# j-min/HiREST

Hardware: AMD Instinct MI355X
Metric: encoded frames/sec (EVA-CLIP-g/14 224^2) (higher is better)
Workload: dtype bf16

## Files before the change

### hirest_amd/_lib.py

```python
from __future__ import annotations

import ctypes as C
import os

HERE = os.path.dirname(os.path.abspath(__file__))
LIB_PATH = os.path.join(HERE, "lib", "libhirest_hip.so")
if os.environ.get("HIREST_LIB_VARIANT"):
    LIB_PATH = os.path.join(HERE, "lib", f"libhirest_hip.{os.environ['HIREST_LIB_VARIANT']}.so")

(EPI_BIAS_BF16, EPI_BIAS_GELU_BF16, EPI_BIAS_QGELU_BF16, EPI_BIAS_RESID_F32, EPI_BIAS_F32, EPI_PATCH_POS_F32,
 EPI_BIAS_RESID_LNSTATS_F32, EPI_LNFOLD_BF16, EPI_LNFOLD_GELU_BF16, EPI_BIAS_GELU_SPLIT2, EPI_BIAS_RESID2_LNSTATS) = range(11)

TOWER_NO_LNFOLD = 1
TOWER_NO_PRUNE = 2
TOWER_F32_RESIDUAL = 4
GEMM_REVERSE = 1
GEMM_X3 = 2
GEMM_X3_T128 = 4
ABI_VERSION = 4

ERRORS = {-1: "HIREST_E_BADARG", -2: "HIREST_E_SHAPE (unsupported shape)", -3: "HIREST_E_WORKSPACE (workspace too small)"}


class GemmArgs(C.Structure):
    _fields_ = [("struct_size", C.c_uint64),
                ("A", C.c_void_p), ("lda", C.c_int64), ("W", C.c_void_p), ("ldw", C.c_int64),
                ("bias", C.c_void_p), ("out", C.c_void_p), ("ldo", C.c_int64),
                ("M", C.c_int32), ("N", C.c_int32), ("K", C.c_int32), ("epilogue", C.c_int32),
                ("pos", C.c_void_p), ("patches_per_frame", C.c_int32), ("aux0", C.c_void_p), ("aux1", C.c_void_p), ("flags", C.c_int32)]

    @classmethod
    def make(cls, *fields):
        return cls(C.sizeof(cls), *fields)



class BlockWeights(C.Structure):
    _fields_ = [(n, C.c_void_p) for n in ("ln1_g", "ln1_b", "qkv_w", "qkv_b", "proj_w", "proj_b",
                                          "ln2_g", "ln2_b", "fc1_w", "fc1_b", "fc2_w", "fc2_b",
                                          "qkv_wf", "qkv_bf", "qkv_s", "fc1_wf", "fc1_bf", "fc1_s")]


class VisionTower(C.Structure):
    _fields_ = [(n, C.c_int32) for n in ("image_size", "patch", "width", "heads", "head_dim", "mlp_dim",
                                         "layers", "embed_dim", "kpad", "act")] + \
               [("ln_eps", C.c_float)] + \
               [("patch_w", C.c_void_p), ("patch_b", C.c_void_p), ("cls", C.c_void_p), ("pos", C.c_void_p),
                ("blocks", C.POINTER(BlockWeights)),
                ("norm_g", C.c_void_p), ("norm_b", C.c_void_p), ("head_w", C.c_void_p), ("head_b", C.c_void_p),
                ("image_mean", C.c_void_p), ("image_std", C.c_void_p),
                ("ln_pre_g", C.c_void_p), ("ln_pre_b", C.c_void_p), ("out_all_tokens", C.c_int32)]


class TextTower(C.Structure):
    _fields_ = [(n, C.c_int32) for n in ("context", "vocab", "width", "heads", "layers", "embed_dim", "act")] + \
               [("ln_eps", C.c_float)] + \
               [("tok_emb", C.c_void_p), ("pos", C.c_void_p), ("blocks", C.POINTER(BlockWeights)),
                ("lnf_g", C.c_void_p), ("lnf_b", C.c_void_p), ("proj_w", C.c_void_p)]


class BlockWeightsF32(C.Structure):
    _fields_ = [(n, C.c_void_p) for n in ("ln1_g", "ln1_b", "qkv_w", "qkv_b", "proj_w", "proj_b",
                                          "ln2_g", "ln2_b", "fc1_w", "fc1_b", "fc2_w", "fc2_b")]


class VisionTowerF32(C.Structure):
    _fields_ = [(n, t) if n != "blocks" else (n, C.POINTER(BlockWeightsF32)) for n, t in VisionTower._fields_]


class TextTowerF32(C.Structure):
    _fields_ = [(n, t) if n != "blocks" else (n, C.POINTER(BlockWeightsF32)) for n, t in TextTower._fields_]


class BlockWeightsX3(C.Structure):
    _fields_ = [(n, C.c_void_p) for n in ("qkv_w2", "proj_w2", "fc1_w2", "fc2_w2")]


class VisionTowerX3(C.Structure):
    _fields_ = [("base", C.POINTER(VisionTowerF32)), ("blocks", C.POINTER(BlockWeightsX3))]


class CaptionLayer(C.Structure):
    _fields_ = [(n, C.c_void_p) for n in ("qkv_w", "qkv_b", "so_w", "so_b", "so_ln_g", "so_ln_b", "cq_w", "cq_b",
                                          "co_w", "co_b", "co_ln_g", "co_ln_b", "ff1_w", "ff1_b", "ff2_w", "ff2_b", "ff_ln_g", "ff_ln_b")]


class CaptionDecoder(C.Structure):
    _fields_ = [(n, C.c_int32) for n in ("layers", "heads", "hidden", "inter", "vocab_padded", "max_pos")] + \
               [(n, C.c_void_p) for n in ("word_emb", "pos_emb", "emb_ln_g", "emb_ln_b")] + \
               [("layer", C.POINTER(CaptionLayer))] + \
               [(n, C.c_void_p) for n in ("tr_w", "tr_b", "tr_ln_g", "tr_ln_b", "lm_w", "lm_b", "lm_w2")]


class JointLayerX3(C.Structure):
    _fields_ = [(n, C.c_void_p) for n in ("qkv_w2", "qkv_b", "ao_w2", "ao_b", "ln1_g", "ln1_b", "fc1_w2", "fc1_b", "fc2_w2", "fc2_b", "ln2_g", "ln2_b")]


class JointEncoderX3(C.Structure):
    _fields_ = [("struct_size", C.c_uint64)] + [(n, C.c_int32) for n in ("layers", "heads", "width", "mlp_dim", "in_dim", "max_pos")] + \
               [("ln_eps", C.c_float), ("attn_shift", C.c_float)] + \
               [(n, C.c_void_p) for n in ("emb_w2", "emb_b", "pos", "emb_ln_g", "emb_ln_b")] + [("layer", C.POINTER(JointLayerX3))]


class ColsumItem(C.Structure):
    _fields_ = [("x", C.c_void_p), ("row_weight", C.c_void_p), ("row_select", C.c_void_p), ("out", C.c_void_p), ("ldx", C.c_int64),
                ("R", C.c_int32), ("C", C.c_int32), ("select_value", C.c_int32), ("reserved", C.c_int32)]


COLSUM_GROUP_MAX = 40


class SplitItem(C.Structure):
    _fields_ = [("x", C.c_void_p), ("out", C.c_void_p), ("ldx", C.c_int64), ("ldo", C.c_int64), ("rows", C.c_int32), ("cols", C.c_int32),
                ("transposed", C.c_int32), ("reserved", C.c_int32)]


class OptimItem(C.Structure):
    _fields_ = [("p", C.c_void_p), ("g", C.c_void_p), ("m", C.c_void_p), ("v", C.c_void_p), ("n", C.c_int64)]


OPTIM_GROUP_MAX = 64
OPTIM_CHUNK = 8192


class TrainBlock(C.Structure):
    _fields_ = [("struct_size", C.c_uint64)] + [(n, C.c_int32) for n in ("B", "T", "heads", "width", "mlp", "precision")] + \
               [("ln_eps", C.c_float), ("drop", C.c_float)] + [(n, C.c_uint32) for n in ("seed_attn", "seed_ao", "seed_out", "reserved")] + \
               [(n, C.c_void_p) for n in ("wqkv", "bqkv", "wo", "bo", "ln1_g", "ln1_b", "w1", "b1", "w2", "b2", "ln2_g", "ln2_b", "x",
                                          "qkv", "P", "cx", "a_pre", "aa", "hpre", "hh", "x_pre", "out", "x2", "out2",
                                          "wqkv2", "wo2", "w12", "w22", "wqkvT2", "woT2", "w1T2", "w2T2", "ws")] + [("ws_bytes", C.c_size_t)]


class TrainFusionBwd(C.Structure):
    _fields_ = [("struct_size", C.c_uint64)] + \
               [(n, C.c_int32) for n in ("B", "T", "E", "W", "vis_dim", "text_dim", "asr_dim", "boundary", "max_pos", "reserved")] + \
               [("drop", C.c_float), ("seed_emb", C.c_uint32)] + \
               [(n, C.c_void_p) for n in ("w_emb", "emb_ln_g", "t2_w", "asr1_w", "asr0_g", "norm_g",
                                          "x0", "f", "v", "tn", "tin", "a0", "asr2", "v0", "vis2", "t", "text", "mm32", "bm32", "n_valid", "dx",
                                          "g_emb_ln_g", "g_emb_ln_b", "g_pos", "g_w_emb", "g_b_emb", "g_mask", "g_bound", "g_t2_w", "g_t2_b", "g_t0_w", "g_t0_b",
                                          "g_asr1_w", "g_asr1_b", "g_asr0_g", "g_asr0_b", "g_norm_g", "g_norm_b", "g_vis_w", "g_vis_b", "g_text_w", "g_text_b")] + \
               [("items", C.POINTER(ColsumItem)), ("n_items", C.POINTER(C.c_int32)), ("max_items", C.c_int32), ("reserved2", C.c_int32),
                ("ws", C.c_void_p), ("ws_bytes", C.c_size_t), ("side_stream", C.c_void_p), ("side_ws", C.c_void_p), ("side_ws_bytes", C.c_size_t),
                ("scratch", C.c_void_p), ("scratch_bytes", C.c_size_t)]


class TrainBlockGrads(C.Structure):
    _fields_ = [("struct_size", C.c_uint64)] + \
               [(n, C.c_void_p) for n in ("dout", "dx", "g_wqkv", "g_wo", "g_w1", "g_w2", "g_bqkv", "g_bo", "g_b1", "g_b2", "g_ln1_g", "g_ln1_b",
                                          "g_ln2_g", "g_ln2_b")] + \
               [("items", C.POINTER(ColsumItem)), ("n_items", C.POINTER(C.c_int32)), ("max_items", C.c_int32), ("reserved", C.c_int32),
                ("side_stream", C.c_void_p), ("side_ws", C.c_void_p), ("side_ws_bytes", C.c_size_t), ("scratch", C.c_void_p),
                ("scratch_bytes", C.c_size_t)]


class JpegImage(C.Structure):
    _fields_ = [(n, C.c_int32) for n in ("width", "height", "ncomp", "hs", "vs", "restart_interval", "mcux", "mcuy", "supported",
                                         "reason")] + \
               [("scan_begin", C.c_int64), ("scan_end", C.c_int64), ("table_set", C.c_int32), ("reserved", C.c_int32),
                ("data_offset", C.c_int64), ("out_offset", C.c_int64), ("ws_offset", C.c_int64),
                ("plane_offset", C.c_int64)]


class JpegTables(C.Structure):
    _fields_ = [("qt", (C.c_uint16 * 64) * 3), ("huff_bits", (C.c_uint8 * 16) * 6), ("huff_vals", (C.c_uint8 * 256) * 6)]


JPEG_REASONS = {0: "ok", 1: "not a JPEG / malformed markers", 2: "progressive", 3: "arithmetic coding", 4: "lossless / hierarchical",
                5: "not 8-bit", 6: "colour space (CMYK / YCCK / RGB / component count)", 7: "sampling factors", 8: "multi-scan",
                9: "truncated (no EOI after the scan)", 10: "bad or missing tables", 11: "image size"}
JPEG_STATUS = {1: "bad Huffman code", 2: "more than 64 coefficients in a block", 4: "out of data", 8: "RSTn out of sequence",
               16: "unsupported"}


BATCH_GATHER_MAX = 8


class BatchGather(C.Structure):
    _fields_ = [("src", C.c_void_p), ("dst", C.c_void_p), ("row_of_example", C.c_void_p), ("words", C.c_int32), ("reserved", C.c_int32)]


class BatchArgs(C.Structure):
    _fields_ = [("struct_size", C.c_uint64), ("index", C.c_void_p)] + \
               [(n, C.c_int32) for n in ("B", "T", "D", "Da", "n_examples", "n_model_frames", "n_gather", "reserved")] + \
               [(n, C.c_void_p) for n in ("frames", "frame_off", "asr_rows", "sub_off", "sub_span", "ex_video", "ex_len", "ex_range",
                                          "bound_off", "bound_val", "vis", "asr", "vis_mask", "moment_mask", "prev_boundary_mask")] + \
               [("gather", BatchGather * BATCH_GATHER_MAX)]


class ProfRecord(C.Structure):
    _fields_ = [("kind", C.c_int32), ("tag", C.c_int32), ("d0", C.c_int64), ("d1", C.c_int64), ("d2", C.c_int64),
                ("ms", C.c_float)]


_SIGNATURES = {
    "hirest_profile_enable": (C.c_int, [C.c_int32]),
    "hirest_attention_debug_mode": (C.c_int, [C.c_int32]),
    "hirest_profile_collect": (C.c_int, [C.POINTER(ProfRecord), C.c_int32]),
    "hirest_abi_version": (C.c_int, []),
    "hirest_build_info": (C.c_char_p, []),
    "hirest_gemm_bf16": (C.c_int, [C.POINTER(GemmArgs), C.c_void_p]),
    "hirest_gemm_select_kernel": (C.c_int, [C.c_int32]),
    "hirest_gemm_debug_mode": (C.c_int, [C.c_int32]),
    "hirest_gemm_dispatch_name": (C.c_int, [C.POINTER(GemmArgs), C.c_char_p, C.c_int32]),
    "hirest_attention_select_kernel": (C.c_int, [C.c_int32]),
    "hirest_attention_set_skew": (C.c_int, [C.c_int32]),
    "hirest_attention_set_mapping": (C.c_int, [C.c_int32]),
    "hirest_attention_set_pace": (C.c_int, [C.c_int32]),
    "hirest_attention_x3_select_waves": (C.c_int, [C.c_int32]),
    "hirest_attention_x3_debug_trace": (C.c_int, [C.c_void_p]),
    "hirest_attention_set_stagger": (C.c_int, [C.c_int32]),
    "hirest_attention_debug_trace_read": (C.c_int, [C.c_void_p, C.c_int32]),
    "hirest_layernorm": (C.c_int, [C.c_void_p, C.c_int64, C.c_void_p, C.c_void_p, C.c_void_p, C.c_float,
                                   C.c_void_p, C.c_int64, C.c_int32, C.c_int32, C.c_int32, C.c_void_p]),
    "hirest_attention_bf16": (C.c_int, [C.c_void_p, C.c_void_p, C.c_int32, C.c_int32, C.c_int32, C.c_int32,
                                        C.c_float, C.c_int32, C.c_void_p]),
    "hirest_attention_bf16_rows": (C.c_int, [C.c_void_p, C.c_void_p, C.c_int32, C.c_int32, C.c_int32, C.c_int32,
                                             C.c_float, C.c_int32, C.c_int32, C.c_void_p]),
    "hirest_fold_layernorm": (C.c_int, [C.c_void_p, C.c_void_p, C.c_void_p, C.c_void_p, C.c_void_p, C.c_void_p, C.c_void_p, C.c_int32,
                                        C.c_int32, C.c_void_p]),
    "hirest_patchify": (C.c_int, [C.c_void_p, C.c_int32, C.c_int32, C.c_int32, C.c_int32, C.c_void_p, C.c_void_p,
                                  C.c_void_p, C.c_int32, C.c_void_p]),
    "hirest_rowstats_bf16": (C.c_int, [C.c_void_p, C.c_int64, C.c_void_p, C.c_void_p, C.c_float, C.c_int32, C.c_int32, C.c_void_p, C.c_void_p]),
    "hirest_rowstats_split_bf16": (C.c_int, [C.c_void_p, C.c_int64, C.c_void_p, C.c_void_p, C.c_void_p, C.c_float, C.c_int32, C.c_int32, C.c_void_p,
                                             C.c_void_p]),
    "hirest_combine_hi_lo_f32": (C.c_int, [C.c_void_p, C.c_void_p, C.c_int64, C.c_void_p, C.c_int64, C.c_int32, C.c_int32, C.c_void_p]),
    "hirest_ln_stats_finalize": (C.c_int, [C.c_void_p, C.c_int32, C.c_void_p, C.c_float, C.c_int32, C.c_int32, C.c_void_p, C.c_void_p]),
    "hirest_write_cls_rows": (C.c_int, [C.c_void_p, C.c_int64, C.c_void_p, C.c_void_p, C.c_int32, C.c_int32,
                                        C.c_int32, C.c_void_p]),
    "hirest_embed_tokens": (C.c_int, [C.c_void_p, C.c_void_p, C.c_void_p, C.c_void_p, C.c_void_p, C.c_int32,
                                      C.c_int32, C.c_int32, C.c_int32, C.c_void_p]),
    "hirest_f32_to_bf16": (C.c_int, [C.c_void_p, C.c_void_p, C.c_int64, C.c_void_p]),
    "hirest_pool_l2norm": (C.c_int, [C.c_void_p, C.c_void_p, C.c_int32, C.c_int32, C.c_int32, C.c_int32, C.c_void_p]),
    "hirest_pool_l2norm_varlen": (C.c_int, [C.c_void_p, C.c_void_p, C.c_void_p, C.c_int32, C.c_int32, C.c_void_p]),
    "hirest_similarity_f32": (C.c_int, [C.c_void_p, C.c_void_p, C.c_void_p, C.c_int32, C.c_int32, C.c_int32, C.c_void_p]),
    "hirest_topk_workspace_bytes": (C.c_int64, [C.c_int32, C.c_int32, C.c_int32]),
    "hirest_topk_f32_ws": (C.c_int, [C.c_void_p, C.c_void_p, C.c_int32, C.c_int32, C.c_int32, C.c_void_p, C.c_void_p, C.c_void_p,
                                     C.c_int64, C.c_void_p]),
    "hirest_topk_f32": (C.c_int, [C.c_void_p, C.c_void_p, C.c_int32, C.c_int32, C.c_int32, C.c_void_p, C.c_void_p,
                                  C.c_void_p]),
    "hirest_clip_score": (C.c_int, [C.c_void_p, C.c_int32, C.c_int32, C.c_void_p, C.c_int32, C.c_void_p, C.c_int32, C.c_int32,
                                    C.c_int32, C.c_void_p, C.c_void_p]),
    "hirest_bertscore_greedy": (C.c_int, [C.c_void_p, C.c_int64, C.c_int32, C.c_void_p, C.c_int32, C.c_void_p, C.c_void_p, C.c_void_p,
                                          C.c_int32, C.c_void_p, C.c_void_p]),
    "hirest_gemm_f32": (C.c_int, [C.c_void_p, C.c_int64, C.c_void_p, C.c_int64, C.c_void_p, C.c_void_p, C.c_int64, C.c_void_p,
                                  C.c_int32, C.c_void_p, C.c_int64, C.c_int32, C.c_int32, C.c_int32, C.c_int32, C.c_void_p]),
    "hirest_attention_f32": (C.c_int, [C.c_void_p, C.c_void_p, C.c_int32, C.c_int32, C.c_int32, C.c_int32, C.c_float,
                                       C.c_float, C.c_void_p]),
    "hirest_attention_f32_qkv": (C.c_int, [C.c_void_p, C.c_int64, C.c_void_p, C.c_void_p, C.c_int64, C.c_void_p, C.c_int32, C.c_int32,
                                           C.c_int32, C.c_int32, C.c_int32, C.c_float, C.c_float, C.c_float, C.c_void_p]),
    "hirest_gemm_f32_select_kernel": (C.c_int, [C.c_int32]),
    "hirest_gemm_f32_workspace_bytes": (C.c_size_t, [C.c_int32, C.c_int32, C.c_int32]),
    "hirest_gemm_f32_layouts_workspace_bytes": (C.c_size_t, [C.c_int32, C.c_int32, C.c_int32]),
    "hirest_gemm_f32_layouts": (C.c_int, [C.c_void_p, C.c_int64, C.c_int32, C.c_void_p, C.c_int64, C.c_int32, C.c_void_p, C.c_void_p, C.c_int64,
                                          C.c_void_p, C.c_int64, C.c_int32, C.c_int32, C.c_int32, C.c_int32, C.c_void_p, C.c_size_t, C.c_void_p]),
    "hirest_gemm_f32_ws": (C.c_int, [C.c_void_p, C.c_int64, C.c_void_p, C.c_int64, C.c_void_p, C.c_void_p, C.c_int64, C.c_void_p,
                                     C.c_int32, C.c_void_p, C.c_int64, C.c_int32, C.c_int32, C.c_int32, C.c_int32, C.c_void_p, C.c_size_t,
                                     C.c_void_p]),
    "hirest_attention_f32_decode": (C.c_int, [C.c_void_p, C.c_int64, C.c_void_p, C.c_void_p, C.c_int64, C.c_void_p, C.c_int32, C.c_void_p,
                                              C.c_void_p, C.c_int64, C.c_void_p, C.c_void_p, C.c_void_p, C.c_int32, C.c_int32, C.c_float,
                                              C.c_float, C.c_float, C.c_void_p]),
    "hirest_gemm_f32_ln": (C.c_int, [C.c_void_p, C.c_int64, C.c_void_p, C.c_void_p, C.c_void_p, C.c_void_p, C.c_void_p, C.c_float,
                                     C.c_void_p, C.c_int64, C.c_void_p, C.c_int64, C.c_void_p, C.c_void_p, C.c_int64, C.c_void_p,
                                     C.c_int64, C.c_int32, C.c_int32, C.c_int32, C.c_int32, C.c_void_p]),
    "hirest_caption_step_workspace_bytes": (C.c_size_t, [C.POINTER(CaptionDecoder), C.c_int32]),
    "hirest_beam_backtrack": (C.c_int, [C.c_void_p, C.c_void_p, C.c_void_p, C.c_void_p, C.c_int32, C.c_int32, C.c_int32, C.c_void_p, C.c_void_p]),
    "hirest_beam_advance": (C.c_int, [C.c_void_p, C.c_void_p, C.c_int32, C.c_int32, C.c_int32, C.c_int32, C.c_int32, C.c_int32,
                                      C.c_void_p, C.c_void_p, C.c_void_p, C.c_void_p, C.c_void_p, C.c_void_p, C.c_void_p, C.c_void_p,
                                      C.c_void_p]),
    "hirest_caption_decode_step": (C.c_int, [C.POINTER(CaptionDecoder), C.c_int32, C.c_int32, C.c_void_p, C.c_void_p,
                                             C.POINTER(C.c_void_p), C.POINTER(C.c_void_p), C.POINTER(C.c_void_p), C.c_int32,
                                             C.c_void_p, C.c_void_p, C.c_void_p, C.c_size_t, C.c_void_p]),
    "hirest_caption_decode_logits": (C.c_int, [C.POINTER(CaptionDecoder), C.c_int32, C.c_int32, C.c_void_p, C.c_void_p,
                                               C.POINTER(C.c_void_p), C.POINTER(C.c_void_p), C.POINTER(C.c_void_p), C.c_int32,
                                               C.c_void_p, C.c_void_p, C.c_size_t, C.c_void_p]),
    "hirest_caption_select": (C.c_int, [C.c_int32]),
    "hirest_gemm_f32_ln_colmax": (C.c_int, [C.c_void_p, C.c_int64, C.c_void_p, C.c_void_p, C.c_float, C.c_void_p, C.c_int64, C.c_void_p,
                                            C.c_void_p, C.c_int64, C.c_void_p, C.c_int32, C.c_int32, C.c_int32, C.c_void_p]),
    "hirest_gemm_f32_rows_ln_mode": (C.c_int, [C.c_int32]),
    "hirest_gemm_f32_ring_mode": (C.c_int, [C.c_int32]),
    "hirest_gemm_f32_rows_preferred": (C.c_int, [C.c_int32]),
    "hirest_gemm_f32_rows_colmax": (C.c_int, [C.c_void_p, C.c_int64, C.c_void_p, C.c_int64, C.c_void_p, C.c_void_p, C.c_int64, C.c_void_p,
                                              C.c_int32, C.c_int32, C.c_int32, C.c_void_p]),
    "hirest_caption_beam_step": (C.c_int, [C.POINTER(CaptionDecoder), C.c_int32, C.c_int32, C.c_int32, C.c_void_p, C.c_void_p,
                                           C.POINTER(C.c_void_p), C.POINTER(C.c_void_p), C.POINTER(C.c_void_p), C.c_int32, C.c_void_p,
                                           C.c_void_p, C.c_int32, C.c_int32, C.c_void_p, C.c_void_p, C.c_void_p, C.c_void_p, C.c_void_p,
                                           C.c_void_p, C.c_void_p, C.c_size_t, C.c_void_p, C.c_size_t, C.c_void_p]),
    "hirest_caption_beam_tail_workspace_bytes": (C.c_size_t, [C.c_int32, C.c_int32, C.c_int32]),
    "hirest_caption_beam_tail": (C.c_int, [C.c_void_p, C.c_int64, C.c_void_p, C.c_int32, C.c_int32, C.c_int32, C.c_int32, C.c_int32,
                                           C.c_int32, C.c_void_p, C.c_void_p, C.c_void_p, C.c_void_p, C.c_void_p, C.c_void_p,
                                           C.c_void_p, C.c_void_p, C.c_void_p, C.c_void_p, C.c_size_t, C.c_void_p]),
    "hirest_attention_f32_varlen": (C.c_int, [C.c_void_p, C.c_void_p, C.c_void_p, C.c_int32, C.c_int32, C.c_int32, C.c_int32, C.c_float,
                                              C.c_float, C.c_void_p]),
    "hirest_log_softmax_f32": (C.c_int, [C.c_void_p, C.c_int64, C.c_void_p, C.c_void_p, C.c_int64, C.c_int32, C.c_int32, C.c_void_p]),
    "hirest_joint_time_grid_f32": (C.c_int, [C.c_void_p, C.c_int32, C.c_int32, C.c_void_p, C.c_void_p]),
    "hirest_joint_time_features": (C.c_int, [C.c_void_p, C.c_void_p, C.c_void_p, C.c_void_p, C.c_int32, C.c_int32, C.c_int32,
                                             C.c_void_p]),
    "hirest_joint_base": (C.c_int, [C.c_void_p, C.c_void_p, C.c_void_p, C.c_void_p, C.c_void_p, C.c_int32, C.c_int32, C.c_int32,
                                    C.c_void_p]),
    "hirest_joint_mask_add": (C.c_int, [C.c_void_p, C.c_void_p, C.c_void_p, C.c_void_p, C.c_void_p, C.c_void_p, C.c_int64,
                                        C.c_int32, C.c_void_p]),
    "hirest_transpose_pad_f32": (C.c_int, [C.c_void_p, C.c_int64, C.c_int32, C.c_int32, C.c_void_p, C.c_int32, C.c_void_p]),
    "hirest_weighted_colsum_grouped_f32": (C.c_int, [C.c_void_p, C.c_int32, C.c_void_p]),
    "hirest_train_fusion_backward_scratch_bytes": (C.c_size_t, [C.POINTER(TrainFusionBwd)]),
    "hirest_train_fusion_backward": (C.c_int, [C.POINTER(TrainFusionBwd), C.c_void_p]),
    "hirest_train_block_forward_scratch_bytes": (C.c_size_t, [C.POINTER(TrainBlock)]),
    "hirest_train_block_forward": (C.c_int, [C.POINTER(TrainBlock), C.c_void_p, C.c_size_t, C.c_void_p]),
    "hirest_train_block_backward_scratch_bytes": (C.c_size_t, [C.POINTER(TrainBlock)]),
    "hirest_train_block_backward": (C.c_int, [C.POINTER(TrainBlock), C.POINTER(TrainBlockGrads), C.c_void_p]),
    "hirest_optim_partials_count": (C.c_int64, [C.c_void_p, C.c_int32]),
    "hirest_grad_sqnorm_grouped_f32": (C.c_int, [C.c_void_p, C.c_int32, C.c_void_p, C.c_void_p]),
    "hirest_clip_coef_f32": (C.c_int, [C.c_void_p, C.c_int64, C.c_float, C.c_void_p, C.c_void_p]),
    "hirest_adamw_grouped_f32": (C.c_int, [C.c_void_p, C.c_int32, C.c_void_p, C.c_float, C.c_float, C.c_float, C.c_float, C.c_float,
                                           C.c_float, C.c_float, C.c_void_p]),
    "hirest_grad_sqnorm_scaled_grouped_f32": (C.c_int, [C.c_void_p, C.c_int32, C.c_void_p, C.c_void_p, C.c_void_p]),
    "hirest_clip_coef_dev_f32": (C.c_int, [C.c_void_p, C.c_int64, C.c_void_p, C.c_void_p, C.c_void_p]),
    "hirest_optim_step_advance_f32": (C.c_int, [C.c_void_p, C.c_int32, C.c_void_p, C.c_void_p]),
    "hirest_adamw_capturable_grouped_f32": (C.c_int, [C.c_void_p, C.c_void_p, C.c_int32, C.c_void_p, C.c_void_p, C.c_double, C.c_void_p,
                                                      C.c_void_p, C.c_double, C.c_double, C.c_float, C.c_double, C.c_void_p]),
    "hirest_weighted_colsum_f32": (C.c_int, [C.c_void_p, C.c_int64, C.c_void_p, C.c_void_p, C.c_int32, C.c_int32, C.c_int32, C.c_void_p, C.c_void_p]),
    "hirest_scale_by_device_scalar_f32": (C.c_int, [C.c_void_p, C.c_void_p, C.c_int64, C.c_void_p]),
    "hirest_act_f32": (C.c_int, [C.c_void_p, C.c_void_p, C.c_int64, C.c_int32, C.c_void_p]),
    "hirest_act_bwd_f32": (C.c_int, [C.c_void_p, C.c_void_p, C.c_void_p, C.c_int64, C.c_int32, C.c_void_p]),
    "hirest_dropout_add_f32": (C.c_int, [C.c_void_p, C.c_void_p, C.c_void_p, C.c_int64, C.c_float, C.c_uint32, C.c_void_p]),
    "hirest_layernorm_bwd_f32": (C.c_int, [C.c_void_p, C.c_void_p, C.c_void_p, C.c_float, C.c_void_p, C.c_void_p, C.c_int32, C.c_int32, C.c_void_p]),
    "hirest_attention_train_select": (C.c_int, [C.c_int32]),
    "hirest_gemm_f32_strided": (C.c_int, [C.c_void_p, C.c_int64, C.c_int64, C.c_void_p, C.c_int64, C.c_int64, C.c_void_p, C.c_int64,
                                          C.c_int32, C.c_int32, C.c_int32, C.c_float, C.c_void_p]),
    "hirest_attention_train_fwd_f32": (C.c_int, [C.c_void_p, C.c_void_p, C.c_void_p, C.c_int32, C.c_int32, C.c_int32, C.c_int32, C.c_float,
                                                 C.c_float, C.c_float, C.c_uint32, C.c_void_p]),
    "hirest_attention_train_bwd_f32": (C.c_int, [C.c_void_p, C.c_void_p, C.c_void_p, C.c_void_p, C.c_void_p, C.c_int32, C.c_int32, C.c_int32,
                                                 C.c_int32, C.c_float, C.c_float, C.c_uint32, C.c_void_p]),
    "hirest_attention_train_fwd_qkv_f32": (C.c_int, [C.c_void_p, C.c_int64, C.c_void_p, C.c_void_p, C.c_int64, C.c_void_p, C.c_void_p, C.c_void_p,
                                                     C.c_int64, C.c_int32, C.c_int32, C.c_int32, C.c_int32, C.c_int32, C.c_float, C.c_float,
                                                     C.c_float, C.c_uint32, C.c_void_p]),
    "hirest_attention_train_bwd_qkv_f32": (C.c_int, [C.c_void_p, C.c_int64, C.c_void_p, C.c_void_p, C.c_int64, C.c_void_p, C.c_void_p, C.c_int64,
                                                     C.c_void_p, C.c_void_p, C.c_int64, C.c_void_p, C.c_void_p, C.c_int64, C.c_int32, C.c_int32,
                                                     C.c_int32, C.c_int32, C.c_int32, C.c_float, C.c_float, C.c_uint32, C.c_void_p]),
    "hirest_embedding_fwd_f32": (C.c_int, [C.c_void_p, C.c_void_p, C.c_void_p, C.c_void_p, C.c_int64, C.c_int32, C.c_int32, C.c_void_p]),
    "hirest_embedding_pos_fwd_f32": (C.c_int, [C.c_void_p, C.c_void_p, C.c_void_p, C.c_void_p, C.c_void_p, C.c_int64, C.c_int32, C.c_void_p]),
    "hirest_embedding_bwd_f32": (C.c_int, [C.c_void_p, C.c_void_p, C.c_void_p, C.c_int64, C.c_int32, C.c_void_p]),
    "hirest_ce_rows_f32": (C.c_int, [C.c_void_p, C.c_int64, C.c_void_p, C.c_int32, C.c_int32, C.c_float, C.c_int32, C.c_void_p, C.c_void_p, C.c_void_p]),
    "hirest_bce_masked_f32": (C.c_int, [C.c_void_p, C.c_void_p, C.c_void_p, C.c_int32, C.c_int32, C.c_float, C.c_void_p, C.c_void_p, C.c_void_p]),
    "hirest_joint_base_bwd_f32": (C.c_int, [C.c_void_p, C.c_void_p, C.c_void_p, C.c_void_p, C.c_void_p, C.c_int32, C.c_int32, C.c_int32, C.c_void_p]),
    "hirest_l2norm_bwd_f32": (C.c_int, [C.c_void_p, C.c_void_p, C.c_void_p, C.c_int32, C.c_int32, C.c_void_p]),
    "hirest_ce_masked_f32": (C.c_int, [C.c_void_p, C.c_void_p, C.c_void_p, C.c_int32, C.c_int32, C.c_float, C.c_void_p, C.c_void_p, C.c_void_p]),
    "hirest_heads_bwd_f32": (C.c_int, [C.c_void_p, C.c_int64, C.c_int32, C.c_int32, C.c_void_p, C.c_void_p, C.c_void_p, C.c_void_p, C.c_void_p]),
    "hirest_linear_heads": (C.c_int, [C.c_void_p, C.c_int64, C.c_int32, C.c_int32, C.c_void_p, C.c_void_p, C.c_void_p, C.c_void_p,
                                      C.c_void_p, C.c_void_p]),
    "hirest_masked_argmax": (C.c_int, [C.c_void_p, C.c_void_p, C.c_float, C.c_int32, C.c_int32, C.c_void_p, C.c_void_p]),
    "hirest_moment_valid_f32": (C.c_int, [C.c_void_p, C.c_void_p, C.c_void_p, C.c_void_p, C.c_void_p, C.c_int32, C.c_int32, C.c_float,
                                          C.c_void_p, C.c_void_p, C.c_void_p]),
    "hirest_lm_head_ce_workspace_bytes": (C.c_size_t, [C.c_int32, C.c_int32]),
    "hirest_lm_head_ce_f32": (C.c_int, [C.c_void_p, C.c_int64, C.c_void_p, C.c_int64, C.c_void_p, C.c_void_p, C.c_int32, C.c_int32,
                                        C.c_int32, C.c_int32, C.c_void_p, C.c_void_p, C.c_void_p, C.c_size_t, C.c_void_p]),
    "hirest_segmentation_step": (C.c_int, [C.c_void_p, C.c_void_p, C.c_void_p, C.c_int32, C.c_int32, C.c_double, C.c_void_p,
                                           C.c_void_p, C.c_int32, C.c_void_p, C.c_void_p]),
    "hirest_preprocess_plan_bytes": (C.c_int64, [C.c_int32, C.c_int32, C.c_int32]),
    "hirest_preprocess_plan": (C.c_int, [C.c_int32, C.c_int32, C.c_int32, C.c_void_p, C.c_int64]),
    "hirest_preprocess_workspace_bytes": (C.c_int64, [C.c_int32, C.c_int32, C.c_int32, C.c_int32]),
    "hirest_preprocess_u8": (C.c_int, [C.c_void_p, C.c_int32, C.c_int32, C.c_int32, C.c_int32, C.c_void_p, C.c_void_p,
                                       C.c_int32, C.c_void_p, C.c_void_p, C.c_void_p, C.c_int64, C.c_void_p]),
    "hirest_jpeg_parse": (C.c_int, [C.c_void_p, C.c_int64, C.POINTER(JpegImage), C.POINTER(JpegTables)]),
    "hirest_jpeg_workspace_bytes": (C.c_int64, [C.POINTER(JpegImage), C.c_int32]),
    "hirest_jpeg_decode": (C.c_int, [C.c_void_p, C.c_void_p, C.c_int32, C.c_void_p, C.c_void_p, C.c_void_p, C.c_void_p, C.c_void_p,
                                     C.c_int64, C.c_void_p]),
    "hirest_jpeg_decode_host": (C.c_int, [C.POINTER(JpegImage), C.POINTER(JpegTables), C.c_void_p, C.c_void_p, C.POINTER(C.c_int32)]),
    "hirest_jpeg_chunked_workspace_bytes": (C.c_int64, [C.c_int32]),
    "hirest_jpeg_decode_chunked": (C.c_int, [C.c_void_p, C.c_void_p, C.c_int32, C.c_void_p, C.c_void_p, C.c_void_p, C.c_void_p, C.c_void_p,
                                             C.c_int64, C.c_int64, C.c_void_p, C.c_int64, C.c_void_p]),
    "hirest_jpeg_decode_host_chunked": (C.c_int, [C.POINTER(JpegImage), C.POINTER(JpegTables), C.c_void_p, C.c_int64, C.c_void_p,
                                                  C.POINTER(C.c_int32), C.POINTER(C.c_int32)]),
    "hirest_interval_iou_f64": (C.c_int, [C.c_void_p, C.c_void_p, C.c_int64, C.c_void_p, C.c_void_p]),
    "hirest_step_bound_pr": (C.c_int, [C.c_void_p, C.c_void_p, C.c_void_p, C.c_void_p, C.c_int32, C.c_double, C.c_void_p,
                                       C.c_void_p, C.c_void_p, C.c_void_p]),
    "hirest_frame_to_timestamp": (C.c_int, [C.c_void_p, C.c_void_p, C.c_void_p, C.c_int32, C.c_int64, C.c_int64, C.c_void_p, C.c_void_p]),
    "hirest_timestamp_to_frame": (C.c_int, [C.c_void_p, C.c_void_p, C.c_void_p, C.c_int32, C.c_int64, C.c_int64, C.c_void_p, C.c_void_p]),
    "hirest_preprocess_moment_bounds": (C.c_int, [C.c_void_p, C.c_void_p, C.c_void_p, C.c_int32, C.c_void_p, C.c_void_p,
                                                  C.c_int32, C.c_void_p]),
    "hirest_cascade_moment_bounds": (C.c_int, [C.c_void_p, C.c_void_p, C.c_void_p, C.c_int32, C.c_int32, C.c_int32, C.c_void_p, C.c_void_p,
                                               C.c_void_p, C.c_void_p, C.c_void_p]),
    "hirest_cascade_boundaries": (C.c_int, [C.c_void_p, C.c_void_p, C.c_void_p, C.c_void_p, C.c_void_p, C.c_int32, C.c_int32, C.c_int32,
                                            C.c_void_p, C.c_void_p, C.c_void_p, C.c_void_p, C.c_void_p, C.c_void_p, C.c_void_p]),
    "hirest_cascade_trim_gather": (C.c_int, [C.c_void_p, C.c_void_p, C.c_void_p, C.c_void_p, C.c_int32, C.c_int32, C.c_int32, C.c_int32,
                                             C.c_int32, C.c_int32, C.c_void_p, C.c_void_p, C.c_void_p]),
    "hirest_batch_assemble": (C.c_int, [C.POINTER(BatchArgs), C.c_void_p]),
    "hirest_vision_workspace_bytes": (C.c_size_t, [C.POINTER(VisionTower), C.c_int32]),
    "hirest_vision_forward": (C.c_int, [C.POINTER(VisionTower), C.c_void_p, C.c_int32, C.c_int32, C.c_void_p,
                                        C.c_void_p, C.c_size_t, C.c_int32, C.c_void_p]),
    "hirest_vision_guard_offset": (C.c_size_t, [C.POINTER(VisionTower), C.c_int32]),
    "hirest_vision_workspace_bytes_f32": (C.c_size_t, [C.POINTER(VisionTowerF32), C.c_int32]),
    "hirest_vision_embed_f32": (C.c_int, [C.POINTER(VisionTowerF32), C.c_void_p, C.c_int32, C.c_int32, C.c_void_p, C.c_void_p, C.c_void_p]),
    "hirest_joint_encoder_x3_workspace_bytes": (C.c_size_t, [C.POINTER(JointEncoderX3), C.c_int32, C.c_int32]),
    "hirest_joint_encoder_x3_forward": (C.c_int, [C.POINTER(JointEncoderX3), C.c_void_p, C.c_int32, C.c_int32, C.c_void_p, C.c_void_p, C.c_size_t,
                                                  C.c_void_p]),
    "hirest_layernorm_f32_split2": (C.c_int, [C.c_void_p, C.c_int64, C.c_void_p, C.c_int32, C.c_void_p, C.c_void_p, C.c_float, C.c_void_p, C.c_int64,
                                              C.c_void_p, C.c_int64, C.c_int32, C.c_int32, C.c_void_p]),
    "hirest_split2_bf16": (C.c_int, [C.c_void_p, C.c_int64, C.c_void_p, C.c_int64, C.c_int64, C.c_int32, C.c_int32, C.c_void_p]),
    "hirest_split2_grouped_bf16": (C.c_int, [C.c_void_p, C.c_int32, C.c_void_p]),
    "hirest_split2_transposed_bf16": (C.c_int, [C.c_void_p, C.c_int64, C.c_void_p, C.c_int64, C.c_int32, C.c_int32, C.c_void_p]),
    "hirest_layernorm_split2": (C.c_int, [C.c_void_p, C.c_int64, C.c_void_p, C.c_void_p, C.c_float, C.c_void_p, C.c_int64, C.c_int32,
                                          C.c_int32, C.c_void_p]),
    "hirest_attention_x3_qkv": (C.c_int, [C.c_void_p, C.c_int64, C.c_void_p, C.c_void_p, C.c_int64, C.c_void_p, C.c_int32, C.c_int32, C.c_int32,
                                          C.c_int32, C.c_int32, C.c_float, C.c_void_p]),
    "hirest_attention_x3_qkv_split2": (C.c_int, [C.c_void_p, C.c_int64, C.c_void_p, C.c_void_p, C.c_int64, C.c_void_p, C.c_int32, C.c_int32,
                                                 C.c_int32, C.c_int32, C.c_int32, C.c_float, C.c_void_p]),
    "hirest_vision_x3_select_attention": (C.c_int, [C.c_int32]),
    "hirest_vision_workspace_bytes_x3": (C.c_size_t, [C.POINTER(VisionTowerX3), C.c_int32]),
    "hirest_vision_forward_x3": (C.c_int, [C.POINTER(VisionTowerX3), C.c_void_p, C.c_int32, C.c_int32, C.c_void_p, C.c_void_p, C.c_size_t,
                                           C.c_void_p]),
    "hirest_vision_forward_f32": (C.c_int, [C.POINTER(VisionTowerF32), C.c_void_p, C.c_int32, C.c_int32, C.c_void_p,
                                            C.c_void_p, C.c_size_t, C.c_void_p]),
    "hirest_text_workspace_bytes_f32": (C.c_size_t, [C.POINTER(TextTowerF32), C.c_int32]),
    "hirest_text_forward_f32": (C.c_int, [C.POINTER(TextTowerF32), C.c_void_p, C.c_int32, C.c_void_p, C.c_void_p,
                                          C.c_size_t, C.c_void_p]),
    "hirest_text_workspace_bytes": (C.c_size_t, [C.POINTER(TextTower), C.c_int32]),
    "hirest_text_forward": (C.c_int, [C.POINTER(TextTower), C.c_void_p, C.c_int32, C.c_void_p, C.c_void_p,
                                      C.c_size_t, C.c_void_p]),
}

EXPORTS = tuple(_SIGNATURES)
_lib = None


def load():
    global _lib
    if _lib is not None:
        return _lib
    if not os.path.isfile(LIB_PATH):
        raise RuntimeError(f"{LIB_PATH} is missing: build it with `python -m hirest_amd.build` "
                           "(hipcc --offload-arch=gfx950). There is no CPU fallback.")
    lib = C.CDLL(LIB_PATH)
    lib.hirest_abi_version.restype, lib.hirest_abi_version.argtypes = C.c_int, []
    if lib.hirest_abi_version() != ABI_VERSION:
        raise RuntimeError(f"libhirest_hip.so ABI version {lib.hirest_abi_version()} != binding {ABI_VERSION}: rebuild with "
                           "`python -m hirest_amd.build --force`")
    for name, (res, args) in _SIGNATURES.items():
        fn = getattr(lib, name)
        fn.restype, fn.argtypes = res, args
    if os.environ.get("HIREST_ATTENTION_KERNEL"):
        check(lib.hirest_attention_select_kernel(int(os.environ["HIREST_ATTENTION_KERNEL"])), "HIREST_ATTENTION_KERNEL")
    _lib = lib
    return lib


def check(code: int, what: str):
    if code == 0:
        return
    if code < 0:
        raise RuntimeError(f"{what}: {ERRORS.get(code, code)}")
    raise RuntimeError(f"{what}: HIP error {code}")
```

### hirest_amd/csrc/attention.hip

```cpp
#include "common.h"
#include <atomic>
#include "profile.h"

namespace {

template <int DH, int DP, int NT>
struct AttnCfg {
    static constexpr int NPAD = 16 * NT;
    static constexpr int KS = (NT + 1) / 2;
    static constexpr int KP = 32 * KS;
    static constexpr int KRS = DP * 2 + 16;
    static constexpr int VRS = KP * 2 + 16;
    static constexpr int LDS_BYTES = NPAD * KRS + DP * VRS;
};

template <int DH, int DP, int NT>
__global__ __launch_bounds__(512) void attention_kernel(const bf16_t* __restrict__ qkv, bf16_t* __restrict__ out,
                                                       int N, int H, float scale_log2e, int causal) {
    using C = AttnCfg<DH, DP, NT>;
    extern __shared__ __attribute__((aligned(16))) char smem[];
    char* Ks = smem;
    char* Vt = smem + C::NPAD * C::KRS;
    const int tid = threadIdx.x, lane = tid & 63, wave = tid >> 6;
    const int b = blockIdx.x / H, h = blockIdx.x - b * H;
    const int D = H * DH;
    const int64_t ld = 3 * (int64_t)D;
    const bf16_t* base = qkv + (int64_t)b * N * ld + h * DH;

    constexpr int KCH = DP / 8;
    for (int idx = tid; idx < C::NPAD * KCH; idx += 512) {
        const int key = idx / KCH, ch = idx - key * KCH;
        bf16x8 v = {0, 0, 0, 0, 0, 0, 0, 0};
        if (key < N && ch * 8 < DH) v = *reinterpret_cast<const bf16x8*>(base + (int64_t)key * ld + D + ch * 8);
        *reinterpret_cast<bf16x8*>(Ks + key * C::KRS + ch * 16) = v;
    }
    constexpr int VCH = DH / 8;
    for (int idx = tid; idx < C::KP * VCH; idx += 512) {
        const int ch = idx / C::KP, key = idx - ch * C::KP;
        bf16x8 v = {0, 0, 0, 0, 0, 0, 0, 0};
        if (key < N) v = *reinterpret_cast<const bf16x8*>(base + (int64_t)key * ld + 2 * D + ch * 8);
#pragma unroll
        for (int e = 0; e < 8; ++e) *reinterpret_cast<bf16_t*>(Vt + (ch * 8 + e) * C::VRS + key * 2) = v[e];
    }
    __syncthreads();

    const int g = lane >> 4, c16 = lane & 15;
    const int nqt = (N + 15) >> 4;
    for (int qt = wave; qt < nqt; qt += 8) {
        const int q = qt * 16 + c16;
        const bool qvalid = q < N;
        bf16x8 qf[DP / 32];
#pragma unroll
        for (int kk = 0; kk < DP / 32; ++kk) {
            const int d = (kk * 4 + g) * 8;
            bf16x8 v = {0, 0, 0, 0, 0, 0, 0, 0};
            if (qvalid && d < DH) v = *reinterpret_cast<const bf16x8*>(base + (int64_t)q * ld + d);
            qf[kk] = v;
        }
        f32x4 st[NT];
#pragma unroll
        for (int t = 0; t < NT; ++t) {
            f32x4 acc = {0.f, 0.f, 0.f, 0.f};
#pragma unroll
            for (int kk = 0; kk < DP / 32; ++kk) {
                const bf16x8 kf = *reinterpret_cast<const bf16x8*>(Ks + (t * 16 + c16) * C::KRS + (kk * 4 + g) * 16);
                acc = __builtin_amdgcn_mfma_f32_16x16x32_bf16(kf, qf[kk], acc, 0, 0, 0);
            }
            st[t] = acc;
            if ((t & 1) == 1) __builtin_amdgcn_sched_barrier(0);
        }
        const int klimit = causal ? (q < N - 1 ? q : N - 1) : N - 1;
        float mx = -3.0e38f;
#pragma unroll
        for (int t = 0; t < NT; ++t)
#pragma unroll
            for (int i = 0; i < 4; ++i) {
                const int key = t * 16 + 4 * g + i;
                const float s = key <= klimit ? st[t][i] : -3.0e38f;
                st[t][i] = s;
                mx = fmaxf(mx, s);
            }
        mx = fmaxf(mx, __shfl_xor(mx, 16, 64));
        mx = fmaxf(mx, __shfl_xor(mx, 32, 64));
        float sum = 0.f;
#pragma unroll
        for (int t = 0; t < NT; ++t)
#pragma unroll
            for (int i = 0; i < 4; ++i) {
                const float pz = exp2f((st[t][i] - mx) * scale_log2e);
                st[t][i] = pz;
                sum += pz;
            }
        sum += __shfl_xor(sum, 16, 64);
        sum += __shfl_xor(sum, 32, 64);
        const float inv = 1.0f / sum;
        bf16x8 pf[C::KS];
#pragma unroll
        for (int s = 0; s < C::KS; ++s) {
#pragma unroll
            for (int i = 0; i < 4; ++i) {
                pf[s][i] = (bf16_t)st[2 * s][i];
                if (2 * s + 1 < NT) pf[s][4 + i] = (bf16_t)st[2 * s + 1][i];
                else pf[s][4 + i] = (bf16_t)0.f;
            }
        }
#pragma unroll 1
        for (int dt = 0; dt < DP / 16; ++dt) {
            f32x4 acc = {0.f, 0.f, 0.f, 0.f};
            const char* vrow = Vt + (dt * 16 + c16) * C::VRS + 8 * g;
#pragma unroll
            for (int s = 0; s < C::KS; ++s) {
                const bf16x4 lo = *reinterpret_cast<const bf16x4*>(vrow + s * 64);
                const bf16x4 hi = *reinterpret_cast<const bf16x4*>(vrow + s * 64 + 32);
                const bf16x8 vf = {lo[0], lo[1], lo[2], lo[3], hi[0], hi[1], hi[2], hi[3]};
                acc = __builtin_amdgcn_mfma_f32_16x16x32_bf16(vf, pf[s], acc, 0, 0, 0);
            }
            const int d = dt * 16 + 4 * g;
            if (qvalid && d < DH) {
                bf16x4 o;
#pragma unroll
                for (int i = 0; i < 4; ++i) o[i] = (bf16_t)(acc[i] * inv);
                *reinterpret_cast<bf16x4*>(out + ((int64_t)b * N + q) * D + h * DH + d) = o;
            }
        }
    }
}

template <int DH, int DP, int NT>
int launch(const bf16_t* qkv, bf16_t* out, int B, int N, int H, float scale, int causal, hipStream_t s) {
    using C = AttnCfg<DH, DP, NT>;
    static HirestDevCfg cfg;
    auto kern = attention_kernel<DH, DP, NT>;
    if (int e = hirest_configure(kern, C::LDS_BYTES, cfg)) return e;
    hipLaunchKernelGGL(kern, dim3(B * H), dim3(512), C::LDS_BYTES, s, qkv, out, N, H, scale * 1.44269504088896340736f, causal);
    return hirest_launch_status();
}


template <int DH, int DP, int NT>
struct AttnCfg2 {
    static constexpr int NPAD = 16 * NT;
    static constexpr int KS = (NT + 1) / 2;
    static constexpr int KP = 32 * KS;
    static constexpr int RS = DP * 2;
    static constexpr int CPR = DP / 8;
    static constexpr int NK_INSTR = NPAD * CPR / 64;
    static constexpr int NV_INSTR = KP * CPR / 64;
    static constexpr int LDS_BYTES = (NPAD + KP) * RS;
};

__device__ __forceinline__ void wait_vm_le(int n) {
    switch (n) {
        case 0: asm volatile("s_waitcnt vmcnt(0)" ::: "memory"); break;
        case 1: asm volatile("s_waitcnt vmcnt(1)" ::: "memory"); break;
        case 2: asm volatile("s_waitcnt vmcnt(2)" ::: "memory"); break;
        case 3: asm volatile("s_waitcnt vmcnt(3)" ::: "memory"); break;
        case 4: asm volatile("s_waitcnt vmcnt(4)" ::: "memory"); break;
        case 5: asm volatile("s_waitcnt vmcnt(5)" ::: "memory"); break;
        case 6: asm volatile("s_waitcnt vmcnt(6)" ::: "memory"); break;
        case 7: asm volatile("s_waitcnt vmcnt(7)" ::: "memory"); break;
        default: asm volatile("s_waitcnt vmcnt(8)" ::: "memory"); break;
    }
}

template <int DH, int DP, int NT>
__global__ __launch_bounds__(512) void attention_kernel_v2(const bf16_t* __restrict__ qkv, bf16_t* __restrict__ out,
                                                          int N, int H, float scale_log2e, int causal) {
    using C = AttnCfg2<DH, DP, NT>;
    extern __shared__ __attribute__((aligned(16))) char smem[];
    char* Ks = smem;
    char* Vs = smem + C::NPAD * C::RS;
    const int tid = threadIdx.x, lane = tid & 63;
    const int wave = __builtin_amdgcn_readfirstlane(tid >> 6);
    const int b = blockIdx.x / H, h = blockIdx.x - b * H;
    const int D = H * DH;
    const int64_t ld = 3 * (int64_t)D;
    const bf16_t* base = qkv + (int64_t)b * N * ld + h * DH;

    int nv_mine = 0;
    for (int i = wave; i < C::NK_INSTR; i += 8) {
        const int ci = i * 64 + lane;
        int row = ci / C::CPR, c = ci - row * C::CPR;
        c = (c & ~3) | ((c & 3) ^ ((-(row >> 2)) & 3));
        row = row < N ? row : N - 1;
        c = c * 8 < DH ? c : DH / 8 - 1;
        glds16(base + (int64_t)row * ld + D + c * 8, Ks + i * 1024);
    }
    for (int i = wave; i < C::NV_INSTR; i += 8) {
        const int ci = i * 64 + lane;
        int row = ci / C::CPR, c = ci - row * C::CPR;
        row = row < N ? row : N - 1;
        c = c * 8 < DH ? c : DH / 8 - 1;
        glds16(base + (int64_t)row * ld + 2 * D + c * 8, Vs + i * 1024);
        ++nv_mine;
    }
    wait_vm_le(nv_mine);
    __builtin_amdgcn_s_barrier();

    const int g = lane >> 4, c16 = lane & 15;
    const int gk = g ^ ((-(c16 >> 2)) & 3);
    const int nqt = (N + 15) >> 4;
    bool v_ready = false;
    for (int qt = wave; qt < nqt; qt += 8) {
        const int q = qt * 16 + c16;
        const bool qvalid = q < N;
        bf16x8 qf[DP / 32];
#pragma unroll
        for (int kk = 0; kk < DP / 32; ++kk) {
            const int d = (kk * 4 + g) * 8;
            bf16x8 v = {0, 0, 0, 0, 0, 0, 0, 0};
            if (qvalid && d < DH) v = *reinterpret_cast<const bf16x8*>(base + (int64_t)q * ld + d);
            qf[kk] = v;
        }
        f32x4 st[NT];
#pragma unroll
        for (int t = 0; t < NT; ++t) {
            f32x4 acc = {0.f, 0.f, 0.f, 0.f};
#pragma unroll
            for (int kk = 0; kk < DP / 32; ++kk) {
                const bf16x8 kf = *reinterpret_cast<const bf16x8*>(Ks + (t * 16 + c16) * C::RS + (kk * 4 + gk) * 16);
                acc = __builtin_amdgcn_mfma_f32_16x16x32_bf16(kf, qf[kk], acc, 0, 0, 0);
            }
            st[t] = acc;
            if ((t & 1) == 1) __builtin_amdgcn_sched_barrier(0);
        }
        const int klimit = causal ? (q < N - 1 ? q : N - 1) : N - 1;
        float mx = -3.0e38f;
#pragma unroll
        for (int t = 0; t < NT; ++t)
#pragma unroll
            for (int i = 0; i < 4; ++i) {
                const int key = t * 16 + 4 * g + i;
                const float sv = key <= klimit ? st[t][i] : -3.0e38f;
                st[t][i] = sv;
                mx = fmaxf(mx, sv);
            }
        mx = fmaxf(mx, __shfl_xor(mx, 16, 64));
        mx = fmaxf(mx, __shfl_xor(mx, 32, 64));
        float sum = 0.f;
#pragma unroll
        for (int t = 0; t < NT; ++t)
#pragma unroll
            for (int i = 0; i < 4; ++i) {
                const float pz = exp2f((st[t][i] - mx) * scale_log2e);
                st[t][i] = pz;
                sum += pz;
            }
        sum += __shfl_xor(sum, 16, 64);
        sum += __shfl_xor(sum, 32, 64);
        const float inv = 1.0f / sum;
        bf16x8 pf[C::KS];
#pragma unroll
        for (int s = 0; s < C::KS; ++s) {
#pragma unroll
            for (int i = 0; i < 4; ++i) {
                pf[s][i] = (bf16_t)st[2 * s][i];
                if (2 * s + 1 < NT) pf[s][4 + i] = (bf16_t)st[2 * s + 1][i];
                else pf[s][4 + i] = (bf16_t)0.f;
            }
        }
        if (!v_ready) {
            asm volatile("s_waitcnt vmcnt(0)" ::: "memory");
            __builtin_amdgcn_s_barrier();
            v_ready = true;
        }
        const char* vlane = Vs + (4 * g + (c16 >> 2)) * C::RS + (c16 & 3) * 8;
#pragma unroll 1
        for (int dt = 0; dt < DP / 16; ++dt) {
            f32x4 acc = {0.f, 0.f, 0.f, 0.f};
            const char* vrow = vlane + dt * 32;
#pragma unroll
            for (int s = 0; s < C::KS; ++s) {
                const bf16x4 lo = __builtin_amdgcn_ds_read_tr16_b64_v4bf16(
                    (__attribute__((address_space(3))) bf16x4*)(vrow + s * 32 * C::RS));
                const bf16x4 hi = __builtin_amdgcn_ds_read_tr16_b64_v4bf16(
                    (__attribute__((address_space(3))) bf16x4*)(vrow + (s * 32 + 16) * C::RS));
                const bf16x8 vf = {lo[0], lo[1], lo[2], lo[3], hi[0], hi[1], hi[2], hi[3]};
                acc = __builtin_amdgcn_mfma_f32_16x16x32_bf16(vf, pf[s], acc, 0, 0, 0);
            }
            const int d = dt * 16 + 4 * g;
            if (qvalid && d < DH) {
                bf16x4 o;
#pragma unroll
                for (int i = 0; i < 4; ++i) o[i] = (bf16_t)(acc[i] * inv);
                *reinterpret_cast<bf16x4*>(out + ((int64_t)b * N + q) * D + h * DH + d) = o;
            }
        }
    }
    if (!v_ready) {
        asm volatile("s_waitcnt vmcnt(0)" ::: "memory");
        __builtin_amdgcn_s_barrier();
    }
}


__device__ __forceinline__ void sleep_n(int n) {
    for (int i = 0; i < n; ++i) __builtin_amdgcn_s_sleep(1);
}
template <int NW, int CPR> struct ROWS_PER_PIECE_OK { static constexpr bool value = (NW * 64 % CPR == 0) && ((NW * 64 / CPR) % 8 == 0); };
__device__ __attribute__((aligned(16))) const unsigned short g_attn_ones[8] = {0x3F80, 0x3F80, 0x3F80, 0x3F80, 0x3F80, 0x3F80, 0x3F80, 0x3F80};
__device__ __attribute__((aligned(16))) const unsigned short g_attn_zeros[8] = {0, 0, 0, 0, 0, 0, 0, 0};
constexpr int ATTN_TRACE_STEPS = 64, ATTN_TRACE_WAVES = 12, ATTN_TRACE_SLOTS = 12;
__device__ long long g_attn_trace[ATTN_TRACE_STEPS * ATTN_TRACE_WAVES * ATTN_TRACE_SLOTS];
__device__ __forceinline__ float max3_raw(float a, float b, float c) {
    float r;
    asm("v_max3_f32 %0, %1, %2, %3" : "=v"(r) : "v"(a), "v"(b), "v"(c));
    return r;
}
typedef float f32x2_t __attribute__((ext_vector_type(2)));
template <int DH, int DP, int NT, bool FAST, bool DBG, int NW = 9, bool LEAN = false, bool PROD = false>
__global__ __launch_bounds__((NW + (PROD ? 1 : 0)) * 64) void attention_kernel_v3(const bf16_t* __restrict__ qkv, bf16_t* __restrict__ out,
                                                          int N, int H, float scale_log2e, int causal, int dbg_bits, int nq, int skew,
                                                          int B, int map, int pace, int stagger) {
    const int dbg = DBG ? dbg_bits : 0;
    using C = AttnCfg2<DH, DP, NT>;
    extern __shared__ __attribute__((aligned(16))) char smem[];
    char* Vs = smem + 2 * C::NPAD * C::RS;
    const int tid = threadIdx.x, lane = tid & 63;
    const int wave = __builtin_amdgcn_readfirstlane(tid >> 6);
    const int D = H * DH;
    const int64_t ld = 3 * (int64_t)D;
    int b0, bstep, h0, hstep, nsteps;
    if (map == 0) { b0 = blockIdx.x; bstep = 0; h0 = 0; hstep = 1; nsteps = H; }
    else {
        const int xcd = blockIdx.x & 7, slot = blockIdx.x >> 3, FL = (gridDim.x >> 3) / H;
        h0 = slot % H; hstep = 0; b0 = xcd * FL + slot / H; bstep = 8 * FL;
        nsteps = b0 < B ? (B - b0 + bstep - 1) / bstep : 0;
    }
    if (nsteps == 0) return;
    if (stagger > 0 && blockIdx.x < 256) sleep_n(((blockIdx.x >> 3) & 15) * stagger);
    auto sbase = [&](int st) { return qkv + (int64_t)(b0 + st * bstep) * N * ld + (h0 + st * hstep) * DH; };
    const int g = lane >> 4, c16 = lane & 15;
    const int gk = g ^ ((-(c16 >> 2)) & 3);
    const int nqt = (nq + 15) >> 4;

    const int ci0 = wave * 64 + lane;
    const int row0 = ci0 / C::CPR, col0 = ci0 - row0 * C::CPR;
    constexpr bool VSWAP = C::RS == 192;
    const int vlog = VSWAP ? ((((col0 >> 1) ^ ((row0 >> 2) & 1)) << 1) | (col0 & 1)) : col0;
    const int vc = vlog * 8 < DH ? vlog : DH / 8 - 1;
    static_assert(ROWS_PER_PIECE_OK<NW, C::CPR>::value, "a lane's rows must keep (row >> 2) & 1 from piece to piece");
    static_assert((NW * 64) % C::CPR == 0, "piece stride must be whole rows");
    constexpr int ROWS_PER_PIECE = NW * 64 / C::CPR;
    auto dma_k = [&](int h, char* dst) -> int {
        int n = 0;
        const bf16_t* src = sbase(h) + D;
        for (int i = wave, row = row0; i < C::NK_INSTR; i += NW, row += ROWS_PER_PIECE) {
            int kc = (col0 & ~3) | ((col0 & 3) ^ ((-(row >> 2)) & 3));
            const bool kpad = kc * 8 >= DH;
            kc = kpad ? DH / 8 - 1 : kc;
            const int r = row < N ? row : N - 1;
            const void* from = src + (int64_t)r * ld + kc * 8;
            if (LEAN && DP > DH) from = kpad ? (const void*)g_attn_zeros : from;
            glds16(from, dst + i * 1024);
            ++n;
        }
        return n;
    };
    constexpr bool SUM_IN_MFMA = LEAN && DP > DH;
    const bool vpad = SUM_IN_MFMA && vlog * 8 >= DH;
    auto dma_v = [&](int h) {
        const bf16_t* src = sbase(h) + 2 * D + vc * 8;
        for (int i = wave, row = row0; i < C::NV_INSTR; i += NW, row += ROWS_PER_PIECE) {
            const int r = row < N ? row : N - 1;
            const void* from = src + (int64_t)r * ld;
            if (SUM_IN_MFMA) from = vpad ? (const void*)g_attn_ones : from;
            glds16(from, Vs + i * 1024);
        }
    };
    auto load_q = [&](int h, int qtile, bf16x8 (&dst)[DP / 32]) {
        const int q = qtile * 16 + c16;
        const bf16_t* base = sbase(h);
        if (LEAN && DP > DH) {
            const bf16_t* row = base + (int64_t)(q < N ? q : N - 1) * ld;
#pragma unroll
            for (int kk = 0; kk < DP / 32; ++kk) {
                const int d = (kk * 4 + g) * 8;
                dst[kk] = *reinterpret_cast<const bf16x8*>(row + (d < DH ? d : DH - 8));
            }
            return;
        }
#pragma unroll
        for (int kk = 0; kk < DP / 32; ++kk) {
            const int d = (kk * 4 + g) * 8;
            bf16x8 v = {0, 0, 0, 0, 0, 0, 0, 0};
            if (qtile < nqt && q < N && d < DH) v = *reinterpret_cast<const bf16x8*>(base + (int64_t)q * ld + d);
            dst[kk] = v;
        }
    };

    if (PROD && wave == NW) {
        constexpr int PER = C::CPR / 4;
        static_assert(C::NK_INSTR % PER == 0 && C::NV_INSTR % PER == 0, "whole 16-row groups");
        int prow[PER], pkoff[PER], pvoff[PER];
        bool pkpad[PER], pvpad[PER];
#pragma unroll
        for (int j = 0; j < PER; ++j) {
            const int ci = j * 64 + lane, r = ci / C::CPR, c = ci - r * C::CPR;
            prow[j] = r;
            int kc = (c & ~3) | ((c & 3) ^ ((-(r >> 2)) & 3));
            pkpad[j] = kc * 8 >= DH;
            pkoff[j] = (pkpad[j] ? DH / 8 - 1 : kc) * 8;
            const int vl = VSWAP ? ((((c >> 1) ^ ((r >> 2) & 1)) << 1) | (c & 1)) : c;
            pvpad[j] = SUM_IN_MFMA && vl * 8 >= DH;
            pvoff[j] = (vl * 8 < DH ? vl : DH / 8 - 1) * 8;
        }
        auto issue_k = [&](int st, char* dst, int pace_units) {
            const bf16_t* src = sbase(st) + D;
            for (int it0 = 0; it0 < C::NK_INSTR / PER; ++it0) {
                const int it = map ? (it0 + h0) % (C::NK_INSTR / PER) : it0;
#pragma unroll
                for (int j = 0; j < PER; ++j) {
                    const int row = prow[j] + 16 * it, r = row < N ? row : N - 1;
                    const void* from = src + (int64_t)r * ld + pkoff[j];
                    if (LEAN && DP > DH) from = pkpad[j] ? (const void*)g_attn_zeros : from;
                    glds16(from, dst + (it * PER + j) * 1024);
                    if (pace_units > 0) sleep_n(pace_units);
                }
            }
        };
        auto issue_v = [&](int st) {
            const bf16_t* src = sbase(st) + 2 * D;
            for (int it0 = 0; it0 < C::NV_INSTR / PER; ++it0) {
                const int it = map ? (it0 + h0) % (C::NV_INSTR / PER) : it0;
#pragma unroll
                for (int j = 0; j < PER; ++j) {
                    const int row = prow[j] + 16 * it, r = row < N ? row : N - 1;
                    const void* from = src + (int64_t)r * ld + pvoff[j];
                    if (SUM_IN_MFMA) from = pvpad[j] ? (const void*)g_attn_ones : from;
                    glds16(from, Vs + (it * PER + j) * 1024);
                }
            }
        };
        issue_k(0, smem, 0);
        for (int h = 0; h < nsteps; ++h) {
            asm volatile("s_waitcnt vmcnt(0)" ::: "memory");
            __builtin_amdgcn_s_barrier();
            issue_v(h);
            asm volatile("s_waitcnt vmcnt(0)" ::: "memory");
            __builtin_amdgcn_s_barrier();
            if (h + 1 < nsteps) issue_k(h + 1, smem + ((h + 1) & 1) * (C::NPAD * C::RS), pace);
        }
        asm volatile("s_waitcnt vmcnt(0)" ::: "memory");
        return;
    }

    bf16x8 qa[DP / 32], qb[DP / 32];
    load_q(0, wave, qa);
    load_q(0, wave + NW, qb);
    if (!(dbg & 8) && !PROD) dma_k(0, smem);
    for (int h = 0; h < nsteps; ++h) {
        const char* Ks = smem + (h & 1) * (C::NPAD * C::RS);
        auto stamp = [&](int slot) {
            if (DBG && (dbg & 256) && blockIdx.x == 0 && h < ATTN_TRACE_STEPS) {
                const long long t = __builtin_readcyclecounter();
                if (lane == 0) g_attn_trace[(h * ATTN_TRACE_WAVES + wave) * ATTN_TRACE_SLOTS + slot] = t;
            }
        };
        stamp(10);
        asm volatile("s_waitcnt vmcnt(0)" ::: "memory");
#pragma unroll
        for (int kk = 0; kk < DP / 32; ++kk) { asm volatile("" : "+v"(qa[kk])); asm volatile("" : "+v"(qb[kk])); }
        if (!(dbg & 128)) __builtin_amdgcn_s_barrier();
        stamp(0);
        if (!(dbg & 8) && !PROD) dma_v(h);
        const int nk_next = (h + 1 < nsteps && !(dbg & 8) && !PROD) ? dma_k(h + 1, smem + ((h + 1) & 1) * (C::NPAD * C::RS)) : 0;
        bool v_ready = false;
        auto tile = [&](int qt, bf16x8 (&qf)[DP / 32], int ord) {
            stamp(1 + 4 * ord);
            const int q = qt * 16 + c16;
            const bool qvalid = q < N;
            f32x4 st[NT];
#pragma unroll
            for (int t = 0; t < NT; t += 2) {
                f32x4 a0 = {0.f, 0.f, 0.f, 0.f}, a1 = {0.f, 0.f, 0.f, 0.f};
                if (!(dbg & 1))
#pragma unroll
                for (int kk = 0; kk < DP / 32; ++kk) {
                    const bf16x8 k0 = *reinterpret_cast<const bf16x8*>(Ks + (t * 16 + c16) * C::RS + (kk * 4 + gk) * 16);
                    a0 = __builtin_amdgcn_mfma_f32_16x16x32_bf16(k0, qf[kk], a0, 0, 0, 0);
                    if (t + 1 < NT) {
                        const bf16x8 k1 = *reinterpret_cast<const bf16x8*>(Ks + ((t + 1) * 16 + c16) * C::RS + (kk * 4 + gk) * 16);
                        a1 = __builtin_amdgcn_mfma_f32_16x16x32_bf16(k1, qf[kk], a1, 0, 0, 0);
                    }
                }
                st[t] = a0;
                if (t + 1 < NT) st[t + 1] = a1;
                if ((t & 2) || !FAST) __builtin_amdgcn_sched_barrier(0);
            }
            if (h + 1 < nsteps && !(dbg & 32)) load_q(h + 1, qt, qf);
            stamp(2 + 4 * ord);
            const int klimit = causal ? (q < N - 1 ? q : N - 1) : N - 1;
            float mx = -3.0e38f;
            float sum = 0.f;
            bf16x8 pf[C::KS];
            if (LEAN) {
                float mxb = -3.0e38f;
#pragma unroll
                for (int t = 0; t < NT; ++t) {
                    if (!FAST || t == NT - 1) {
#pragma unroll
                        for (int i = 0; i < 4; ++i) st[t][i] = (t * 16 + 4 * g + i) <= klimit ? st[t][i] : -3.0e38f;
                    }
                    if (t & 1) { mxb = max3_raw(mxb, st[t][0], st[t][1]); mxb = max3_raw(mxb, st[t][2], st[t][3]); }
                    else { mx = max3_raw(mx, st[t][0], st[t][1]); mx = max3_raw(mx, st[t][2], st[t][3]); }
                }
                float pa = max3_raw(mx, mxb, mxb), pb = pa;
                lane_swap16(pa, pb); pa = max3_raw(pa, pb, pb); pb = pa; lane_swap32(pa, pb); mx = max3_raw(pa, pb, pb);
                const float nmc = -mx * scale_log2e;
                const f32x2_t sc2 = {scale_log2e, scale_log2e}, nm2 = {nmc, nmc};
                f32x2_t sum2 = {0.f, 0.f};
#pragma unroll
                for (int s2 = 0; s2 < C::KS; ++s2) {
#pragma unroll
                    for (int u = 0; u < 2; ++u) {
                        if (2 * s2 + u < NT) {
#pragma unroll
                            for (int ip = 0; ip < 2; ++ip) {
                                const f32x2_t sv = {st[2 * s2 + u][2 * ip], st[2 * s2 + u][2 * ip + 1]};
                                const f32x2_t e = __builtin_elementwise_fma(sv, sc2, nm2);
                                const f32x2_t p2 = (dbg & 2) ? e : f32x2_t{__builtin_amdgcn_exp2f(e[0]), __builtin_amdgcn_exp2f(e[1])};
                                if (!SUM_IN_MFMA) sum2 += p2;
                                pf[s2][4 * u + 2 * ip] = (bf16_t)p2[0];
                                pf[s2][4 * u + 2 * ip + 1] = (bf16_t)p2[1];
                            }
                        } else {
#pragma unroll
                            for (int i = 0; i < 4; ++i) pf[s2][4 + i] = (bf16_t)0.f;
                        }
                    }
                }
                if (!SUM_IN_MFMA) {
                    sum = sum2[0] + sum2[1];
                    float sa = sum, sb = sum; lane_swap16(sa, sb); sum = sa + sb; sa = sum; sb = sum; lane_swap32(sa, sb); sum = sa + sb;
                }
            } else {
#pragma unroll
            for (int t = 0; t < NT; ++t) {
                if (!FAST || t == NT - 1) {
#pragma unroll
                    for (int i = 0; i < 4; ++i) st[t][i] = (t * 16 + 4 * g + i) <= klimit ? st[t][i] : -3.0e38f;
                }
                mx = fmaxf(fmaxf(mx, fmaxf(st[t][0], st[t][1])), fmaxf(st[t][2], st[t][3]));
            }
            { float pa = mx, pb = mx; lane_swap16(pa, pb); mx = fmaxf(pa, pb); pa = mx; pb = mx; lane_swap32(pa, pb); mx = fmaxf(pa, pb); }
            const float nmc = -mx * scale_log2e;
#pragma unroll
            for (int s2 = 0; s2 < C::KS; ++s2) {
#pragma unroll
                for (int i = 0; i < 4; ++i) {
                    const float e0 = fmaf(st[2 * s2][i], scale_log2e, nmc);
                    const float p0 = (dbg & 2) ? e0 : __builtin_amdgcn_exp2f(e0);
                    sum += p0;
                    pf[s2][i] = (bf16_t)p0;
                    if (2 * s2 + 1 < NT) {
                        const float e1 = fmaf(st[2 * s2 + 1][i], scale_log2e, nmc);
                        const float p1 = (dbg & 2) ? e1 : __builtin_amdgcn_exp2f(e1);
                        sum += p1;
                        pf[s2][4 + i] = (bf16_t)p1;
                    } else {
                        pf[s2][4 + i] = (bf16_t)0.f;
                    }
                }
            }
            { float pa = sum, pb = sum; lane_swap16(pa, pb); sum = pa + pb; pa = sum; pb = sum; lane_swap32(pa, pb); sum = pa + pb; }
            }
            stamp(3 + 4 * ord);
            if (!v_ready) {
                if (!PROD) wait_vm_le(nk_next);
                if (!(dbg & 64)) __builtin_amdgcn_s_barrier();
                v_ready = true;
            }
            stamp(4 + 4 * ord);
            const char* vlane = Vs + (4 * g + (c16 >> 2)) * C::RS + (c16 & 3) * 8;
            const char* vl_e = vlane + ((VSWAP && (g & 1)) ? 32 : 0);
            const char* vl_o = vlane - ((VSWAP && (g & 1)) ? 32 : 0);
            f32x4 oacc[DP / 16];
#pragma unroll
            for (int dt = 0; dt < DP / 16; ++dt) oacc[dt] = f32x4{0.f, 0.f, 0.f, 0.f};
            if (!(dbg & 4))
#pragma unroll
            for (int s2 = 0; s2 < C::KS; ++s2) {
#pragma unroll
                for (int dt = 0; dt < DP / 16; ++dt) {
                    const char* vrow = ((dt & 1) ? vl_o : vl_e) + dt * 32 + s2 * 32 * C::RS;
                    const bf16x4 lo = __builtin_amdgcn_ds_read_tr16_b64_v4bf16((__attribute__((address_space(3))) bf16x4*)(vrow));
                    const bf16x4 hi = __builtin_amdgcn_ds_read_tr16_b64_v4bf16((__attribute__((address_space(3))) bf16x4*)(vrow + 16 * C::RS));
                    const bf16x8 vf = {lo[0], lo[1], lo[2], lo[3], hi[0], hi[1], hi[2], hi[3]};
                    oacc[dt] = __builtin_amdgcn_mfma_f32_16x16x32_bf16(vf, pf[s2], oacc[dt], 0, 0, 0);
                }
                if ((s2 & 1) || !FAST) __builtin_amdgcn_sched_barrier(0);
            }
            if (SUM_IN_MFMA) {
                float sa = oacc[DP / 16 - 1][0], sb = sa;
                lane_swap32(sa, sb);
                sum = sb;
            }
            const float inv = 1.0f / sum;
            static_assert((DP / 16) % 2 == 0 && DH % 8 == 0, "paired d tiles");
#pragma unroll
            for (int dp = 0; dp < DP / 32; ++dp) {
                union { bf16x4 v; unsigned u[2]; } e, o;
#pragma unroll
                for (int i = 0; i < 4; ++i) { e.v[i] = (bf16_t)(oacc[2 * dp][i] * inv); o.v[i] = (bf16_t)(oacc[2 * dp + 1][i] * inv); }
                const auto s0 = __builtin_amdgcn_permlane16_swap(e.u[0], o.u[0], false, false);
                const auto s1 = __builtin_amdgcn_permlane16_swap(e.u[1], o.u[1], false, false);
                union { bf16x8 v; unsigned u[4]; } w;
                w.u[0] = s0[0]; w.u[1] = s1[0]; w.u[2] = s0[1]; w.u[3] = s1[1];
                const int d = (2 * dp + (g & 1)) * 16 + (g >> 1) * 8;
                if (qvalid && d < DH && !(dbg & 16)) *reinterpret_cast<bf16x8*>(out + ((int64_t)(b0 + h * bstep) * N + q) * D + (h0 + h * hstep) * DH + d) = w.v;
            }
        };
        if (skew > 0 && wave >= 4 && wave < 8) sleep_n(skew);
        if (wave < nqt) tile(wave, qa, 0);
        if (wave + NW < nqt) tile(wave + NW, qb, 1);
        stamp(9);
        if (!v_ready) {
            if (!PROD) wait_vm_le(nk_next);
            __builtin_amdgcn_s_barrier();
        }
    }
    asm volatile("s_waitcnt vmcnt(0)" ::: "memory");
}

std::atomic<int> g_attn_dbg{0};
std::atomic<int> g_attn_skew{12};
std::atomic<int> g_attn_stagger{16};
std::atomic<int> g_attn_pace{0};
std::atomic<int> g_attn_map{2};
std::atomic<int> g_attn_variant{7};

template <int DH, int DP, int NT, bool FAST, bool DBG, int NW = 9, bool LEAN = false, bool PROD = false>
int launch3_impl(const bf16_t* qkv, bf16_t* out, int B, int N, int H, float scale, int causal, int nq, hipStream_t s) {
    using C = AttnCfg2<DH, DP, NT>;
    constexpr int LDS = (2 * C::NPAD + C::KP) * C::RS;
    static_assert(LDS <= 163840, "K x2 + V must fit the CU's LDS");
    static HirestDevCfg cfg;
    auto kern = attention_kernel_v3<DH, DP, NT, FAST, DBG, NW, LEAN, PROD>;
    if (int e = hirest_configure(kern, LDS, cfg)) return e;
    const bool by_head = (g_attn_map == 1 || (g_attn_map == 2 && B < 256)) && H <= 32 && 32 % H == 0 && B >= 8 * (32 / H) * 4;
    const int grid = by_head ? 256 : B;
    hipLaunchKernelGGL(kern, dim3(grid), dim3((NW + (PROD ? 1 : 0)) * 64), LDS, s, qkv, out, N, H, scale * 1.44269504088896340736f, causal, g_attn_dbg, nq,
                       g_attn_skew, B, by_head ? 1 : 0, g_attn_pace, g_attn_stagger);
    return hirest_launch_status();
}

template <int DH, int DP, int NT, bool FAST>
int launch3(const bf16_t* qkv, bf16_t* out, int B, int N, int H, float scale, int causal, int nq, hipStream_t s) {
    if (g_attn_dbg && FAST && g_attn_variant == 6) return launch3_impl<DH, DP, NT, FAST, true, 9, true, true>(qkv, out, B, N, H, scale, causal, nq, s);
    if (g_attn_variant == 6) return launch3_impl<DH, DP, NT, FAST, false, 9, true, true>(qkv, out, B, N, H, scale, causal, nq, s);
    if (g_attn_dbg && FAST && g_attn_variant == 7) return launch3_impl<DH, DP, NT, FAST, true, 9, false, true>(qkv, out, B, N, H, scale, causal, nq, s);
    if (g_attn_variant == 7) return launch3_impl<DH, DP, NT, FAST, false, 9, false, true>(qkv, out, B, N, H, scale, causal, nq, s);
    if (g_attn_dbg && FAST && g_attn_variant == 5) return launch3_impl<DH, DP, NT, FAST, true, 9, true>(qkv, out, B, N, H, scale, causal, nq, s);
    if (g_attn_dbg && FAST) return launch3_impl<DH, DP, NT, FAST, true>(qkv, out, B, N, H, scale, causal, nq, s);
    if (g_attn_variant == 4) return launch3_impl<DH, DP, NT, FAST, false, 12>(qkv, out, B, N, H, scale, causal, nq, s);
    if (g_attn_variant == 5) return launch3_impl<DH, DP, NT, FAST, false, 9, true>(qkv, out, B, N, H, scale, causal, nq, s);
    return launch3_impl<DH, DP, NT, FAST, false>(qkv, out, B, N, H, scale, causal, nq, s);
}


template <int DH, int DP, int NT>
int launch2(const bf16_t* qkv, bf16_t* out, int B, int N, int H, float scale, int causal, hipStream_t s) {
    using C = AttnCfg2<DH, DP, NT>;
    static HirestDevCfg cfg;
    auto kern = attention_kernel_v2<DH, DP, NT>;
    if (int e = hirest_configure(kern, C::LDS_BYTES, cfg)) return e;
    hipLaunchKernelGGL(kern, dim3(B * H), dim3(512), C::LDS_BYTES, s, qkv, out, N, H, scale * 1.44269504088896340736f, causal);
    return hirest_launch_status();
}

}

extern "C" int hirest_attention_debug_mode(int32_t bits) { g_attn_dbg = bits; return 0; }

extern "C" int hirest_attention_set_skew(int32_t units) {
    if (units < 0 || units > 64) return HIREST_E_BADARG;
    g_attn_skew = units;
    return 0;
}

extern "C" int hirest_attention_debug_trace_read(int64_t* dst, int32_t n) {
    if (!dst || n <= 0 || n > ATTN_TRACE_STEPS * ATTN_TRACE_WAVES * ATTN_TRACE_SLOTS) return HIREST_E_BADARG;
    return (int)hipMemcpyFromSymbol(dst, HIP_SYMBOL(g_attn_trace), sizeof(long long) * n);
}

extern "C" int hirest_attention_set_stagger(int32_t units) {
    if (units < 0 || units > 64) return HIREST_E_BADARG;
    g_attn_stagger = units;
    return 0;
}

extern "C" int hirest_attention_set_pace(int32_t units) {
    if (units < 0 || units > 64) return HIREST_E_BADARG;
    g_attn_pace = units;
    return 0;
}

extern "C" int hirest_attention_set_mapping(int32_t by_head) {
    if (by_head < 0 || by_head > 2) return HIREST_E_BADARG;
    g_attn_map = by_head;
    return 0;
}

extern "C" int hirest_attention_select_kernel(int32_t which) {
    if (which < 1 || which > 7) return HIREST_E_BADARG;
    g_attn_variant = which;
    return 0;
}

extern "C" int hirest_attention_bf16(const hirest_bf16* qkv, hirest_bf16* out, int32_t B, int32_t N, int32_t H,
                                     int32_t dh, float scale, int32_t causal, void* stream) {
    return hirest_attention_bf16_rows(qkv, out, B, N, H, dh, scale, causal, N, stream);
}

extern "C" int hirest_attention_bf16_rows(const hirest_bf16* qkv, hirest_bf16* out, int32_t B, int32_t N, int32_t H,
                                          int32_t dh, float scale, int32_t causal, int32_t q_rows, void* stream) {
    if (!qkv || !out || B <= 0 || N <= 0 || H <= 0 || q_rows <= 0 || q_rows > N) return HIREST_E_BADARG;
    const int nq = q_rows;
    hipStream_t s = reinterpret_cast<hipStream_t>(stream);
    const bf16_t* q = reinterpret_cast<const bf16_t*>(qkv);
    bf16_t* o = reinterpret_cast<bf16_t*>(out);
    HirestProfScope prof(HIREST_PROF_ATTENTION, causal, (int64_t)B * H, N, dh, s);
    if (g_attn_variant >= 3 && N > 80 && N <= 272 && B >= 64) {
        const bool fast = !causal && N > 256;
        if (dh == 88) return fast ? launch3<88, 96, 17, true>(q, o, B, N, H, scale, causal, nq, s)
                                  : launch3<88, 96, 17, false>(q, o, B, N, H, scale, causal, nq, s);
        if (dh == 64) return fast ? launch3<64, 64, 17, true>(q, o, B, N, H, scale, causal, nq, s)
                                  : launch3<64, 64, 17, false>(q, o, B, N, H, scale, causal, nq, s);
    }
    if (g_attn_variant >= 2) {
        if (dh == 88) {
            if (N <= 80) return launch2<88, 96, 5>(q, o, B, N, H, scale, causal, s);
            if (N <= 272) return launch2<88, 96, 17>(q, o, B, N, H, scale, causal, s);
        } else if (dh == 64) {
            if (N <= 80) return launch2<64, 64, 5>(q, o, B, N, H, scale, causal, s);
            if (N <= 272) return launch2<64, 64, 17>(q, o, B, N, H, scale, causal, s);
        }
        return HIREST_E_SHAPE;
    }
    if (dh == 88) {
        if (N <= 80) return launch<88, 96, 5>(q, o, B, N, H, scale, causal, s);
        if (N <= 272) return launch<88, 96, 17>(q, o, B, N, H, scale, causal, s);
    } else if (dh == 64) {
        if (N <= 80) return launch<64, 64, 5>(q, o, B, N, H, scale, causal, s);
        if (N <= 272) return launch<64, 64, 17>(q, o, B, N, H, scale, causal, s);
    }
    return HIREST_E_SHAPE;
}
```

### hirest_amd/ops.py

```python
from __future__ import annotations

import ctypes as C
import functools
from typing import Optional

import torch

from . import _lib
from ._lib import (EPI_BIAS_BF16, EPI_BIAS_F32, EPI_BIAS_GELU_BF16, EPI_BIAS_QGELU_BF16, EPI_BIAS_RESID_F32,
                   EPI_PATCH_POS_F32)

__all__ = ["gemm", "layernorm", "attention", "patchify", "write_cls_rows", "embed_tokens", "to_bf16",
           "pool_l2norm", "similarity", "topk", "clip_score", "stream_ptr", "on_tensor_device"]


_raw_stream = getattr(torch._C, "_cuda_getCurrentRawStream", None)


def stream_ptr() -> int:
    if _raw_stream is not None:
        return _raw_stream(torch.cuda.current_device())
    return torch.cuda.current_stream().cuda_stream


def on_tensor_device(fn):
    @functools.wraps(fn)
    def wrapped(*args, **kw):
        for a in list(args) + list(kw.values()):
            if isinstance(a, torch.Tensor) and a.is_cuda:
                if a.device.index != torch.cuda.current_device():
                    with torch.cuda.device(a.device):
                        return fn(*args, **kw)
                break
        return fn(*args, **kw)
    return wrapped


def _dev(t: torch.Tensor, dtype, name: str) -> int:
    if not isinstance(t, torch.Tensor) or not t.is_cuda:
        raise RuntimeError(f"{name}: expected a GPU tensor (the HIP path has no CPU fallback)")
    if t.dtype != dtype:
        raise RuntimeError(f"{name}: expected dtype {dtype}, got {t.dtype}")
    if not t.is_contiguous():
        raise RuntimeError(f"{name}: expected a contiguous tensor")
    return t.data_ptr()


def _opt(t: Optional[torch.Tensor], dtype, name: str) -> Optional[int]:
    return None if t is None else _dev(t, dtype, name)


@on_tensor_device
def gemm(a: torch.Tensor, w: torch.Tensor, bias: Optional[torch.Tensor], out: torch.Tensor, epilogue: int,
         pos: Optional[torch.Tensor] = None, patches_per_frame: int = 0,
         aux0: Optional[torch.Tensor] = None, aux1: Optional[torch.Tensor] = None, flags: int = 0) -> torch.Tensor:
    lib = _lib.load()
    M, K = a.shape
    N = w.shape[0]
    if w.shape[1] != K:
        raise RuntimeError(f"gemm: K mismatch {a.shape} x {w.shape}")
    out_dtype = torch.bfloat16 if epilogue in (EPI_BIAS_BF16, EPI_BIAS_GELU_BF16, EPI_BIAS_QGELU_BF16, _lib.EPI_LNFOLD_BF16,
                                              _lib.EPI_LNFOLD_GELU_BF16, _lib.EPI_BIAS_RESID2_LNSTATS) else torch.float32
    args = _lib.GemmArgs.make(_dev(a, torch.bfloat16, "gemm.a"), K, _dev(w, torch.bfloat16, "gemm.w"), K,
                         _opt(bias, torch.float32, "gemm.bias"), _dev(out, out_dtype, "gemm.out"), out.shape[-1],
                         M, N, K, epilogue, _opt(pos, torch.float32, "gemm.pos"), patches_per_frame,
                         None if aux0 is None else _dev(aux0, aux0.dtype, "gemm.aux0"),
                         None if aux1 is None else _dev(aux1, aux1.dtype, "gemm.aux1"), int(flags))
    _lib.check(lib.hirest_gemm_bf16(C.byref(args), stream_ptr()), "hirest_gemm_bf16")
    return out


def gemm_select_kernel(which: int):
    _lib.check(_lib.load().hirest_gemm_select_kernel(int(which)), "hirest_gemm_select_kernel")


ATTENTION_DEFAULT_KERNEL = 7


def attention_select_kernel(which: int):
    _lib.check(_lib.load().hirest_attention_select_kernel(int(which)), "hirest_attention_select_kernel")


def attention_set_mapping(by_head: Optional[bool] = None):
    _lib.check(_lib.load().hirest_attention_set_mapping(2 if by_head is None else int(bool(by_head))), "hirest_attention_set_mapping")


@on_tensor_device
def layernorm(x: torch.Tensor, gamma: torch.Tensor, beta: torch.Tensor, eps: float, out: torch.Tensor,
              row_index: Optional[torch.Tensor] = None, ldx: Optional[int] = None, rows: Optional[int] = None):
    lib = _lib.load()
    D = gamma.numel()
    rows = rows if rows is not None else (row_index.numel() if row_index is not None else x.numel() // D)
    ldx = ldx if ldx is not None else D
    out_f32 = 1 if out.dtype == torch.float32 else 0
    _lib.check(lib.hirest_layernorm(_dev(x, torch.float32, "ln.x"), ldx, _opt(row_index, torch.int32, "ln.row_index"),
                                    _dev(gamma, torch.float32, "ln.gamma"), _dev(beta, torch.float32, "ln.beta"),
                                    float(eps), _dev(out, out.dtype, "ln.out"), D, out_f32, rows, D, stream_ptr()),
               "hirest_layernorm")
    return out


@on_tensor_device
def attention(qkv: torch.Tensor, out: torch.Tensor, B: int, N: int, H: int, dh: int, causal: bool,
              scale: Optional[float] = None):
    lib = _lib.load()
    scale = dh ** -0.5 if scale is None else scale
    _lib.check(lib.hirest_attention_bf16(_dev(qkv, torch.bfloat16, "attn.qkv"), _dev(out, torch.bfloat16, "attn.out"),
                                         B, N, H, dh, float(scale), int(bool(causal)), stream_ptr()),
               "hirest_attention_bf16")
    return out


_IN_DTYPES = {torch.float32: 0, torch.bfloat16: 1, torch.uint8: 2}


@on_tensor_device
def patchify(frames: torch.Tensor, patch: int, kpad: int, out: torch.Tensor, mean=None, std=None):
    lib = _lib.load()
    if frames.dtype not in _IN_DTYPES:
        raise RuntimeError(f"patchify: unsupported frame dtype {frames.dtype}")
    code = _IN_DTYPES[frames.dtype]
    B = frames.shape[0]
    S = frames.shape[-1] if code != 2 else frames.shape[1]
    _lib.check(lib.hirest_patchify(_dev(frames, frames.dtype, "patchify.frames"), code, B, S, patch,
                                   _opt(mean, torch.float32, "mean"), _opt(std, torch.float32, "std"),
                                   _dev(out, torch.bfloat16, "patchify.out"), kpad, stream_ptr()), "hirest_patchify")
    return out


@on_tensor_device
def write_cls_rows(x: torch.Tensor, cls: torch.Tensor, pos0: torch.Tensor, B: int, T: int, D: int):
    lib = _lib.load()
    _lib.check(lib.hirest_write_cls_rows(_dev(x, torch.float32, "x"), D, _dev(cls, torch.float32, "cls"),
                                         _dev(pos0, torch.float32, "pos"), B, T, D, stream_ptr()), "hirest_write_cls_rows")
    return x


@on_tensor_device
def embed_tokens(tokens: torch.Tensor, tok_emb: torch.Tensor, pos: torch.Tensor, x: torch.Tensor, eot_row: torch.Tensor):
    lib = _lib.load()
    B, L = tokens.shape
    V, D = tok_emb.shape
    _lib.check(lib.hirest_embed_tokens(_dev(tokens, torch.int64, "tokens"), _dev(tok_emb, torch.float32, "tok_emb"),
                                       _dev(pos, torch.float32, "pos"), _dev(x, torch.float32, "x"),
                                       _dev(eot_row, torch.int32, "eot_row"), B, L, D, V, stream_ptr()), "hirest_embed_tokens")
    return x


@on_tensor_device
def to_bf16(t: torch.Tensor) -> torch.Tensor:
    lib = _lib.load()
    t = t.contiguous()
    out = torch.empty(t.shape, dtype=torch.bfloat16, device=t.device)
    n = t.numel()
    if n % 4 != 0:
        raise RuntimeError("to_bf16: element count must be a multiple of 4")
    _lib.check(lib.hirest_f32_to_bf16(_dev(t, torch.float32, "to_bf16.in"), out.data_ptr(), n, stream_ptr()), "hirest_f32_to_bf16")
    return out


@on_tensor_device
def split2(x: torch.Tensor, gelu: bool = False) -> torch.Tensor:
    lib = _lib.load()
    rows, D = x.shape
    out = torch.empty((rows, 2 * D), dtype=torch.bfloat16, device=x.device)
    _lib.check(lib.hirest_split2_bf16(_dev(x, torch.float32, "split2.in"), D, out.data_ptr(), 2 * D, rows, D, int(bool(gelu)), stream_ptr()),
               "hirest_split2_bf16")
    return out


@on_tensor_device
def gemm_x3(a2: torch.Tensor, w2: torch.Tensor, bias: Optional[torch.Tensor] = None, resid_out: Optional[torch.Tensor] = None,
            gelu_split: bool = False, stream=None) -> torch.Tensor:
    lib = _lib.load()
    M, K2 = a2.shape
    N = w2.shape[0]
    if gelu_split:
        out = torch.empty((M, 2 * N), dtype=torch.bfloat16, device=a2.device)
        args = _lib.GemmArgs.make(_dev(a2, torch.bfloat16, "gemm_x3.a"), K2, _dev(w2, torch.bfloat16, "gemm_x3.w"), K2,
                                  _opt(bias, torch.float32, "gemm_x3.bias"), out.data_ptr(), 2 * N, M, N, K2, _lib.EPI_BIAS_GELU_SPLIT2, None, 0,
                                  None, None, _lib.GEMM_X3)
        _lib.check(lib.hirest_gemm_bf16(C.byref(args), stream_ptr()), "hirest_gemm_bf16 (x3, gelu + split)")
        return out
    out = resid_out if resid_out is not None else torch.empty((M, N), dtype=torch.float32, device=a2.device)
    epi = _lib.EPI_BIAS_RESID_F32 if resid_out is not None else _lib.EPI_BIAS_F32
    args = _lib.GemmArgs.make(_dev(a2, torch.bfloat16, "gemm_x3.a"), K2, _dev(w2, torch.bfloat16, "gemm_x3.w"), K2,
                              _opt(bias, torch.float32, "gemm_x3.bias"), out.data_ptr(), N, M, N, K2, epi, None, 0, None, None, _lib.GEMM_X3)
    _lib.check(lib.hirest_gemm_bf16(C.byref(args), stream_ptr() if stream is None else stream), "hirest_gemm_bf16 (x3)")
    return out


@on_tensor_device
def pool_l2norm(frame_embeds: torch.Tensor, normalize_frames_first: bool = False) -> torch.Tensor:
    lib = _lib.load()
    V, F, E = frame_embeds.shape
    out = torch.empty((V, E), dtype=torch.float32, device=frame_embeds.device)
    _lib.check(lib.hirest_pool_l2norm(_dev(frame_embeds, torch.float32, "pool.in"), out.data_ptr(), V, F, E,
                                      int(bool(normalize_frames_first)), stream_ptr()), "hirest_pool_l2norm")
    return out


@on_tensor_device
def similarity(text_n: torch.Tensor, video_n: torch.Tensor) -> torch.Tensor:
    lib = _lib.load()
    Q, E = text_n.shape
    V = video_n.shape[0]
    out = torch.empty((Q, V), dtype=torch.float32, device=text_n.device)
    _lib.check(lib.hirest_similarity_f32(_dev(text_n, torch.float32, "sim.text"), _dev(video_n, torch.float32, "sim.video"),
                                         out.data_ptr(), Q, V, E, stream_ptr()), "hirest_similarity_f32")
    return out


def gemm_f32_strided(a: torch.Tensor, b: torch.Tensor, alpha: float = 1.0) -> torch.Tensor:
    lib = _lib.load()
    M, K = a.shape
    N = b.shape[0]
    out = torch.empty((M, N), dtype=torch.float32, device=a.device)
    _lib.check(lib.hirest_gemm_f32_strided(_dev(a, torch.float32, "gemm.a"), a.stride(0), 1, _dev(b, torch.float32, "gemm.b"), b.stride(0), 1,
                                           out.data_ptr(), N, M, N, K, float(alpha), stream_ptr()), "hirest_gemm_f32_strided")
    return out


@on_tensor_device
def topk(scores: torch.Tensor, k: int, tie_rank: Optional[torch.Tensor] = None):
    lib = _lib.load()
    Q, V = scores.shape
    idx = torch.empty((Q, k), dtype=torch.int32, device=scores.device)
    val = torch.empty((Q, k), dtype=torch.float32, device=scores.device)
    if V >= 16384:
        need = lib.hirest_topk_workspace_bytes(Q, V, k)
        ws = torch.empty(need, dtype=torch.uint8, device=scores.device)
        _lib.check(lib.hirest_topk_f32_ws(_dev(scores, torch.float32, "topk.scores"), _opt(tie_rank, torch.int32, "topk.tie_rank"),
                                          Q, V, k, idx.data_ptr(), val.data_ptr(), ws.data_ptr(), need, stream_ptr()),
                   "hirest_topk_f32_ws")
        return val, idx
    _lib.check(lib.hirest_topk_f32(_dev(scores, torch.float32, "topk.scores"), _opt(tie_rank, torch.int32, "topk.tie_rank"),
                                   Q, V, k, idx.data_ptr(), val.data_ptr(), stream_ptr()), "hirest_topk_f32")
    return val, idx



@on_tensor_device
def clip_score(img_rows: torch.Tensor, txt_rows: torch.Tensor, sel) -> torch.Tensor:
    lib = _lib.load()
    if img_rows.dim() != 2 or txt_rows.dim() != 2 or img_rows.shape[1] != txt_rows.shape[1]:
        raise RuntimeError(f"clip_score: expected [U, E] and [C, E] rows, got {tuple(img_rows.shape)} and {tuple(txt_rows.shape)}")
    sel = torch.as_tensor(sel)
    U, E = img_rows.shape
    C = txt_rows.shape[0]
    if sel.dim() != 2 or sel.shape[0] != C or sel.shape[1] < 1:
        raise RuntimeError(f"clip_score: sel must be [C={C}, K>=1], got {tuple(sel.shape)}")
    if sel.numel() and (int(sel.min()) < 0 or int(sel.max()) >= U):
        raise RuntimeError(f"clip_score: row ids must lie in [0, {U})")
    for t, name in ((img_rows, "clip_score.img"), (txt_rows, "clip_score.txt")):
        if t.dtype not in (torch.float32, torch.bfloat16):
            raise RuntimeError(f"{name}: expected fp32 or bf16 rows, got {t.dtype}")
    out = torch.empty(C, dtype=torch.float32, device=img_rows.device)
    sel = sel.to(device=img_rows.device, dtype=torch.int32).contiguous()
    _lib.check(lib.hirest_clip_score(_dev(img_rows, img_rows.dtype, "clip_score.img"), _IN_DTYPES[img_rows.dtype], U,
                                     _dev(txt_rows, txt_rows.dtype, "clip_score.txt"), _IN_DTYPES[txt_rows.dtype],
                                     sel.data_ptr(), C, sel.shape[1], E, out.data_ptr(), stream_ptr()), "hirest_clip_score")
    return out

BERTSCORE_MAX_TOKENS = 1024


@on_tensor_device
def bertscore_greedy(states: torch.Tensor, seq_off, tok_weight: torch.Tensor, cand_seq, ref_seq) -> torch.Tensor:
    lib = _lib.load()
    if not isinstance(states, torch.Tensor) or not states.is_cuda or states.dtype != torch.float32 or states.dim() != 2 \
            or (states.numel() and states.stride(1) != 1):
        raise RuntimeError("bertscore_greedy.states: expected a [tokens, D] fp32 GPU tensor with unit column stride")
    rows, D = states.shape
    ld = states.stride(0) if rows > 1 else D
    seq_off, cand_seq, ref_seq = torch.as_tensor(seq_off), torch.as_tensor(cand_seq), torch.as_tensor(ref_seq)
    if seq_off.dim() != 1 or seq_off.numel() < 2 or cand_seq.dim() != 1 or cand_seq.shape != ref_seq.shape:
        raise RuntimeError("bertscore_greedy: seq_off must be [n_seq + 1 >= 2], cand_seq and ref_seq [n_pairs]")
    if not seq_off.is_cuda:
        lens = seq_off[1:] - seq_off[:-1]
        if int(seq_off[0]) < 0 or int(seq_off[-1]) > rows or int(lens.min()) < 1 or int(lens.max()) > BERTSCORE_MAX_TOKENS:
            raise RuntimeError(f"bertscore_greedy.seq_off: sentences of 1 .. {BERTSCORE_MAX_TOKENS} rows inside the {rows} rows")
    if tok_weight.shape != (rows,):
        raise RuntimeError(f"bertscore_greedy.tok_weight: expected [{rows}], got {tuple(tok_weight.shape)}")
    dev = states.device
    seq_off, cand_seq, ref_seq = (t.to(device=dev, dtype=torch.int32).contiguous() for t in (seq_off, cand_seq, ref_seq))
    n_pairs = cand_seq.numel()
    out = torch.empty((n_pairs, 3), dtype=torch.float32, device=dev)
    if n_pairs == 0:
        return out
    _lib.check(lib.hirest_bertscore_greedy(states.data_ptr(), ld, D, seq_off.data_ptr(), seq_off.numel() - 1,
                                           _dev(tok_weight, torch.float32, "bertscore_greedy.tok_weight"), cand_seq.data_ptr(),
                                           ref_seq.data_ptr(), n_pairs, out.data_ptr(), stream_ptr()), "hirest_bertscore_greedy")
    return out


@on_tensor_device
def moment_valid(logits: torch.Tensor, vis_mask: torch.Tensor, moment_mask: torch.Tensor, start_target: torch.Tensor,
                 end_target: torch.Tensor, fill: float = -1e10):
    lib = _lib.load()
    if vis_mask.dim() != 2 or moment_mask.shape != vis_mask.shape:
        raise ValueError(f"moment_valid: masks must be [B, T], got {tuple(vis_mask.shape)} and {tuple(moment_mask.shape)}")
    B, T = vis_mask.shape
    if B < 1 or T < 1 or tuple(logits.shape) != (2, B * T) or tuple(start_target.shape) != (B,) or tuple(end_target.shape) != (B,):
        raise ValueError(f"moment_valid: expected logits [2, {B * T}] and targets [{B}], got {tuple(logits.shape)}, "
                         f"{tuple(start_target.shape)}, {tuple(end_target.shape)}")
    pred = torch.empty((B, 2), dtype=torch.int32, device=logits.device)
    loss = torch.empty((), dtype=torch.float32, device=logits.device)
    _lib.check(lib.hirest_moment_valid_f32(_dev(logits, torch.float32, "moment_valid.logits"), _dev(vis_mask, torch.int32, "moment_valid.vis_mask"),
                                           _dev(moment_mask, torch.int32, "moment_valid.moment_mask"),
                                           _dev(start_target, torch.int32, "moment_valid.start_target"),
                                           _dev(end_target, torch.int32, "moment_valid.end_target"), B, T, float(fill), pred.data_ptr(),
                                           loss.data_ptr(), stream_ptr()), "hirest_moment_valid_f32")
    return pred, loss


@on_tensor_device
def lm_head_ce(h: torch.Tensor, w: torch.Tensor, bias: torch.Tensor, target: torch.Tensor, n_valid: Optional[int] = None):
    lib = _lib.load()
    if h.dim() != 2 or w.dim() != 2 or h.shape[0] < 1 or w.shape[0] < 1 or h.shape[1] != w.shape[1]:
        raise ValueError(f"lm_head_ce: expected h [R, K] and w [V, K], got {tuple(h.shape)} and {tuple(w.shape)}")
    R, K = h.shape
    V = w.shape[0]
    if tuple(bias.shape) != (V,) or tuple(target.shape) != (R,):
        raise ValueError(f"lm_head_ce: expected bias [{V}] and target [{R}], got {tuple(bias.shape)} and {tuple(target.shape)}")
    n_valid = R if n_valid is None else int(n_valid)
    if n_valid < 0 or n_valid > R:
        raise ValueError(f"lm_head_ce: n_valid must lie in [0, {R}], got {n_valid}")
    need = lib.hirest_lm_head_ce_workspace_bytes(R, V)
    ws = torch.empty(need, dtype=torch.uint8, device=h.device)
    nll = torch.empty((R,), dtype=torch.float32, device=h.device)
    loss = torch.empty((), dtype=torch.float32, device=h.device)
    _lib.check(lib.hirest_lm_head_ce_f32(_dev(h, torch.float32, "lm_head_ce.h"), K, _dev(w, torch.float32, "lm_head_ce.w"), K,
                                         _dev(bias, torch.float32, "lm_head_ce.bias"), _dev(target, torch.int32, "lm_head_ce.target"),
                                         R, V, K, n_valid, nll.data_ptr(), loss.data_ptr(), ws.data_ptr(), need, stream_ptr()),
               "hirest_lm_head_ce_f32")
    return nll, loss


def to_device(t: torch.Tensor, device) -> torch.Tensor:
    if t.device.type == "cpu" and t.is_pinned():
        return t.to(device, non_blocking=True)
    return t.to(device)


_STREAM_WS = {}
_STREAM_WS_RETIRED = []


def stream_workspace(device, nbytes: int, tag=0, stream: Optional[int] = None):
    if nbytes <= 0:
        return None, 0
    key = (device.type, device.index, tag, int(stream) if stream is not None else stream_ptr())
    buf = _STREAM_WS.get(key)
    if buf is None or buf.numel() < nbytes:
        if buf is not None:
            _STREAM_WS_RETIRED.append(buf)
        buf = torch.empty(max(int(nbytes), 2 * (buf.numel() if buf is not None else 0), 32 << 20), dtype=torch.uint8, device=device)
        _STREAM_WS[key] = buf
    return buf.data_ptr(), buf.numel()
```

### include/hirest_hip.h

```cpp
#ifndef HIREST_HIP_H
#define HIREST_HIP_H

#include <stddef.h>
#include <stdint.h>

#ifdef __cplusplus
extern "C" {
#endif

#define HIREST_ABI_VERSION 4

#define HIREST_E_BADARG   (-1)
#define HIREST_E_SHAPE    (-2)
#define HIREST_E_WORKSPACE (-3)

typedef uint16_t hirest_bf16;

int hirest_abi_version(void);
const char* hirest_build_info(void);

enum hirest_epilogue {
    HIREST_EPI_BIAS_BF16 = 0,
    HIREST_EPI_BIAS_GELU_BF16 = 1,
    HIREST_EPI_BIAS_QGELU_BF16 = 2,
    HIREST_EPI_BIAS_RESID_F32 = 3,
    HIREST_EPI_BIAS_F32 = 4,
    HIREST_EPI_PATCH_POS_F32 = 5,
    HIREST_EPI_BIAS_RESID_LNSTATS_F32 = 6,
    HIREST_EPI_LNFOLD_BF16 = 7,
    HIREST_EPI_LNFOLD_GELU_BF16 = 8,
    HIREST_EPI_BIAS_GELU_SPLIT2 = 9,
    HIREST_EPI_BIAS_RESID2_LNSTATS = 10
};

typedef struct hirest_gemm_args {
    uint64_t struct_size;
    const hirest_bf16* A;  int64_t lda;
    const hirest_bf16* W;  int64_t ldw;
    const float* bias;
    void* out;             int64_t ldo;
    int32_t M, N, K;
    int32_t epilogue;
    const float* pos;
    int32_t patches_per_frame;
    void* aux0;
    void* aux1;
    int32_t flags;
} hirest_gemm_args;
enum { HIREST_GEMM_REVERSE = 1,
       HIREST_GEMM_X3 = 2,
       HIREST_GEMM_X3_T128 = 4
     };

int hirest_gemm_bf16(const hirest_gemm_args* args, void* stream);
int hirest_gemm_select_kernel(int32_t which);
int hirest_gemm_debug_mode(int32_t bits);
int hirest_gemm_dispatch_name(const hirest_gemm_args* args, char* out, int32_t out_len);

int hirest_layernorm(const float* x, int64_t ldx, const int32_t* row_index,
                     const float* gamma, const float* beta, float eps,
                     void* out, int64_t ldo, int32_t out_is_f32,
                     int32_t rows, int32_t D, void* stream);

int hirest_attention_bf16(const hirest_bf16* qkv, hirest_bf16* out,
                          int32_t B, int32_t N, int32_t H, int32_t dh,
                          float scale, int32_t causal, void* stream);
int hirest_attention_bf16_rows(const hirest_bf16* qkv, hirest_bf16* out,
                               int32_t B, int32_t N, int32_t H, int32_t dh,
                               float scale, int32_t causal, int32_t q_rows, void* stream);
int hirest_attention_select_kernel(int32_t which);
int hirest_attention_set_mapping(int32_t by_head);
int hirest_attention_set_pace(int32_t units);
int hirest_attention_set_stagger(int32_t units);
int hirest_attention_set_skew(int32_t units);
int hirest_attention_debug_mode(int32_t bits);
int hirest_attention_debug_trace_read(int64_t* dst, int32_t n);

int hirest_patchify(const void* frames, int32_t in_dtype, int32_t B, int32_t S, int32_t P,
                    const float* mean3, const float* std3,
                    hirest_bf16* patches, int32_t Kpad, void* stream);

int hirest_fold_layernorm(const float* W, const float* gamma, const float* beta, const float* bias, hirest_bf16* Wf,
                          float* bias_out, float* colsum_out, int32_t N, int32_t K, void* stream);
int hirest_write_cls_rows(float* x, int64_t ldx, const float* cls, const float* pos0,
                          int32_t B, int32_t tokens_per_frame, int32_t D, void* stream);

int hirest_rowstats_bf16(const float* x, int64_t ldx, hirest_bf16* xb, float* stats, float eps, int32_t rows, int32_t D,
                         float* guard, void* stream);
int hirest_rowstats_split_bf16(const float* x, int64_t ldx, hirest_bf16* xb, hirest_bf16* xlo, float* stats, float eps, int32_t rows,
                               int32_t D, float* guard, void* stream);
int hirest_combine_hi_lo_f32(const hirest_bf16* hi, const hirest_bf16* lo, int64_t ld_in, float* out, int64_t ldo, int32_t rows,
                             int32_t D, void* stream);
int hirest_ln_stats_finalize(const float* partials, int32_t groups, float* stats, float eps, int32_t rows, int32_t D,
                             float* guard, void* stream);

int hirest_embed_tokens(const int64_t* tokens, const float* tok_emb, const float* pos,
                        float* x, int32_t* eot_row, int32_t B, int32_t L, int32_t D,
                        int32_t vocab, void* stream);

int hirest_f32_to_bf16(const float* in, hirest_bf16* out, int64_t n, void* stream);

int hirest_pool_l2norm(const float* frame_embeds, float* out, int32_t V, int32_t F, int32_t E,
                       int32_t normalize_frames_first, void* stream);
int hirest_pool_l2norm_varlen(const float* rows, const int32_t* seg_off, float* out, int32_t V, int32_t E, void* stream);

int hirest_similarity_f32(const float* text_n, const float* video_n, float* scores,
                          int32_t Q, int32_t V, int32_t E, void* stream);

int hirest_topk_f32(const float* scores, const int32_t* tie_rank, int32_t Q, int32_t V, int32_t k,
                    int32_t* out_index, float* out_score, void* stream);
int64_t hirest_topk_workspace_bytes(int32_t Q, int32_t V, int32_t k);
int hirest_topk_f32_ws(const float* scores, const int32_t* tie_rank, int32_t Q, int32_t V, int32_t k,
                       int32_t* out_index, float* out_score, void* workspace, int64_t workspace_bytes, void* stream);
int hirest_clip_score(const void* img_rows, int32_t img_dtype, int32_t U, const void* txt_rows, int32_t txt_dtype,
                      const int32_t* sel, int32_t C, int32_t K, int32_t E, float* out, void* stream);

#define HIREST_BERTSCORE_MAX_TOKENS 1024
int hirest_bertscore_greedy(const float* states, int64_t ld, int32_t D, const int32_t* seq_off, int32_t n_seq,
                            const float* tok_weight, const int32_t* cand_seq, const int32_t* ref_seq, int32_t n_pairs,
                            float* out , void* stream);

typedef struct hirest_block_weights {
    const float* ln1_g; const float* ln1_b;
    const hirest_bf16* qkv_w; const float* qkv_b;
    const hirest_bf16* proj_w; const float* proj_b;
    const float* ln2_g; const float* ln2_b;
    const hirest_bf16* fc1_w; const float* fc1_b;
    const hirest_bf16* fc2_w; const float* fc2_b;
    const hirest_bf16* qkv_wf; const float* qkv_bf; const float* qkv_s;
    const hirest_bf16* fc1_wf; const float* fc1_bf; const float* fc1_s;
} hirest_block_weights;

typedef struct hirest_vision_tower {
    int32_t image_size, patch, width, heads, head_dim, mlp_dim, layers, embed_dim;
    int32_t kpad;
    int32_t act;
    float ln_eps;
    const hirest_bf16* patch_w;
    const float* patch_b;
    const float* cls;
    const float* pos;
    const hirest_block_weights* blocks;
    const float* norm_g; const float* norm_b;
    const hirest_bf16* head_w;
    const float* head_b;
    const float* image_mean; const float* image_std;
    const float* ln_pre_g; const float* ln_pre_b;
    int32_t out_all_tokens;
} hirest_vision_tower;

size_t hirest_vision_workspace_bytes(const hirest_vision_tower* t, int32_t B);
enum { HIREST_TOWER_NO_LNFOLD = 1,
       HIREST_TOWER_NO_PRUNE = 2,
       HIREST_TOWER_F32_RESIDUAL = 4 };
int hirest_vision_forward(const hirest_vision_tower* t, const void* frames, int32_t in_dtype,
                          int32_t B, float* out, void* workspace, size_t workspace_bytes,
                          int32_t flags, void* stream);
size_t hirest_vision_guard_offset(const hirest_vision_tower* t, int32_t B);

typedef struct hirest_text_tower {
    int32_t context, vocab, width, heads, layers, embed_dim;
    int32_t act;
    float ln_eps;
    const float* tok_emb;
    const float* pos;
    const hirest_block_weights* blocks;
    const float* lnf_g; const float* lnf_b;
    const hirest_bf16* proj_w;
} hirest_text_tower;

size_t hirest_text_workspace_bytes(const hirest_text_tower* t, int32_t B);
int hirest_text_forward(const hirest_text_tower* t, const int64_t* tokens, int32_t B, float* out,
                        void* workspace, size_t workspace_bytes, void* stream);

typedef struct hirest_block_weights_f32 {
    const float* ln1_g; const float* ln1_b;
    const float* qkv_w; const float* qkv_b;
    const float* proj_w; const float* proj_b;
    const float* ln2_g; const float* ln2_b;
    const float* fc1_w; const float* fc1_b;
    const float* fc2_w; const float* fc2_b;
} hirest_block_weights_f32;

typedef struct hirest_vision_tower_f32 {
    int32_t image_size, patch, width, heads, head_dim, mlp_dim, layers, embed_dim;
    int32_t kpad;
    int32_t act;
    float ln_eps;
    const float* patch_w;
    const float* patch_b; const float* cls; const float* pos;
    const hirest_block_weights_f32* blocks;
    const float* norm_g; const float* norm_b;
    const float* head_w; const float* head_b;
    const float* image_mean; const float* image_std;
    const float* ln_pre_g; const float* ln_pre_b;
    int32_t out_all_tokens;
} hirest_vision_tower_f32;

typedef struct hirest_text_tower_f32 {
    int32_t context, vocab, width, heads, layers, embed_dim;
    int32_t act;
    float ln_eps;
    const float* tok_emb; const float* pos;
    const hirest_block_weights_f32* blocks;
    const float* lnf_g; const float* lnf_b;
    const float* proj_w;
} hirest_text_tower_f32;

size_t hirest_vision_workspace_bytes_f32(const hirest_vision_tower_f32* t, int32_t B);
int hirest_vision_forward_f32(const hirest_vision_tower_f32* t, const void* frames, int32_t in_dtype, int32_t B, float* out,
                              void* workspace, size_t workspace_bytes, void* stream);
int hirest_vision_embed_f32(const hirest_vision_tower_f32* t, const void* frames, int32_t in_dtype, int32_t B, float* x, float* rows,
                            void* stream);
size_t hirest_text_workspace_bytes_f32(const hirest_text_tower_f32* t, int32_t B);
int hirest_text_forward_f32(const hirest_text_tower_f32* t, const int64_t* tokens, int32_t B, float* out,
                            void* workspace, size_t workspace_bytes, void* stream);

typedef struct hirest_block_weights_x3 {
    const hirest_bf16* qkv_w2;
    const hirest_bf16* proj_w2;
    const hirest_bf16* fc1_w2;
    const hirest_bf16* fc2_w2;
} hirest_block_weights_x3;

typedef struct hirest_vision_tower_x3 {
    const hirest_vision_tower_f32* base;
    const hirest_block_weights_x3* blocks;
} hirest_vision_tower_x3;

int hirest_split2_bf16(const float* x, int64_t ldx, hirest_bf16* out, int64_t ldo, int64_t rows, int32_t D, int32_t act, void* stream);
int hirest_split2_transposed_bf16(const float* x, int64_t ldx, hirest_bf16* out, int64_t ldo, int32_t rows, int32_t cols, void* stream);
#define HIREST_SPLIT_GROUP_MAX 16
typedef struct hirest_split_item {
    const float* x; hirest_bf16* out;
    int64_t ldx, ldo;
    int32_t rows, cols, transposed, reserved;
} hirest_split_item;
int hirest_split2_grouped_bf16(const hirest_split_item* items, int32_t count, void* stream);
int hirest_layernorm_split2(const float* x, int64_t ldx, const float* gamma, const float* beta, float eps, hirest_bf16* out, int64_t ldo,
                            int32_t rows, int32_t D, void* stream);
int hirest_attention_x3_qkv(const float* q, int64_t ldq, const float* k, const float* v, int64_t ldkv, float* out, int32_t B, int32_t Tq,
                            int32_t Tk, int32_t H, int32_t dh, float scale, void* stream);
int hirest_attention_x3_qkv_split2(const float* q, int64_t ldq, const float* k, const float* v, int64_t ldkv, hirest_bf16* out2, int32_t B,
                                   int32_t Tq, int32_t Tk, int32_t H, int32_t dh, float scale, void* stream);
int hirest_attention_x3_select_waves(int32_t waves);
int hirest_attention_x3_debug_trace(int64_t* device_buffer);
int hirest_vision_x3_select_attention(int32_t which);
size_t hirest_vision_workspace_bytes_x3(const hirest_vision_tower_x3* t, int32_t B);
int hirest_vision_forward_x3(const hirest_vision_tower_x3* t, const void* frames, int32_t in_dtype, int32_t B, float* out,
                             void* workspace, size_t workspace_bytes, void* stream);

int hirest_gemm_f32(const float* A, int64_t lda, const float* W, int64_t ldw, const float* bias,
                    const float* resid, int64_t ldr, const float* periodic, int32_t period,
                    float* out, int64_t ldo, int32_t M, int32_t N, int32_t K, int32_t act, void* stream);
size_t hirest_gemm_f32_workspace_bytes(int32_t M, int32_t N, int32_t K);
int hirest_gemm_f32_ws(const float* A, int64_t lda, const float* W, int64_t ldw, const float* bias, const float* resid, int64_t ldr,
                       const float* periodic, int32_t period, float* out, int64_t ldo, int32_t M, int32_t N, int32_t K, int32_t act,
                       void* workspace, size_t workspace_bytes, void* stream);
size_t hirest_gemm_f32_layouts_workspace_bytes(int32_t M, int32_t N, int32_t K);
int hirest_gemm_f32_layouts(const float* A, int64_t lda, int32_t a_kmajor, const float* W, int64_t ldw, int32_t w_kmajor,
                            const float* bias, const float* resid, int64_t ldr, float* out, int64_t ldo, int32_t M, int32_t N,
                            int32_t K, int32_t act, void* workspace, size_t workspace_bytes, void* stream);
int hirest_gemm_f32_select_kernel(int32_t which);
int hirest_gemm_f32_ring_mode(int32_t mode);
int hirest_gemm_f32_ln(const float* X, int64_t ldx, const int32_t* ids, const float* table, const float* pos_row,
                       const float* gamma, const float* beta, float eps, float* ln_out, int64_t ldl, const float* W, int64_t ldw,
                       const float* bias, const float* resid, int64_t ldr, float* out, int64_t ldo, int32_t M, int32_t N, int32_t K,
                       int32_t act, void* stream);
int hirest_gemm_f32_ln_colmax(const float* X, int64_t ldx, const float* gamma, const float* beta, float eps, const float* W, int64_t ldw,
                              const float* bias, float* out, int64_t ldo, float* colmax, int32_t M, int32_t N, int32_t K, void* stream);
int hirest_gemm_f32_rows_ln_mode(int32_t mode);
int hirest_gemm_f32_rows_preferred(int32_t M);
int hirest_gemm_f32_rows_colmax(const float* A, int64_t lda, const float* W, int64_t ldw, const float* bias, float* out, int64_t ldo,
                                float* colmax, int32_t M, int32_t N, int32_t K, void* stream);
int hirest_attention_f32(const float* qkv, float* out, int32_t B, int32_t T, int32_t H, int32_t dh,
                         float scale, float add_const, void* stream);
int hirest_attention_f32_qkv(const float* q, int64_t ldq, const float* k, const float* v, int64_t ldkv, float* out,
                             int32_t B, int32_t Tq, int32_t Tk, int32_t H, int32_t dh, float scale, float add_const,
                             float causal_penalty, void* stream);
int hirest_attention_f32_varlen(const float* qkv, float* out, const int32_t* seq_off, int32_t B, int32_t max_len, int32_t H,
                                int32_t dh, float scale, float add_const, void* stream);
int hirest_log_softmax_f32(const float* x, int64_t ldx, const float* row_add, float* out, int64_t ldo, int32_t rows,
                           int32_t V, void* stream);
int hirest_joint_time_features(const int32_t* n_valid, const float* w1, const float* b1, float* tin,
                               int32_t B, int32_t T, int32_t E, void* stream);
int hirest_joint_time_grid_f32(const int32_t* n_valid, int32_t B, int32_t T, float* grid, void* stream);
int hirest_joint_base(const float* v, const float* text_proj, const float* asr, const float* temporal, float* base,
                      int32_t B, int32_t T, int32_t E, void* stream);
int hirest_joint_mask_add(const float* base, const int32_t* moment_mask, const int32_t* boundary_mask,
                          const float* mask_embed, const float* boundary_embed, float* f, int64_t rows, int32_t E,
                          void* stream);
int hirest_linear_heads(const float* x, int64_t rows, int32_t D, int32_t nheads, const float* w0, const float* w1,
                        const float* w2, const float* bias3, float* logits, void* stream);
typedef struct hirest_caption_layer {
    const float* qkv_w; const float* qkv_b;
    const float* so_w; const float* so_b; const float* so_ln_g; const float* so_ln_b;
    const float* cq_w; const float* cq_b;
    const float* co_w; const float* co_b; const float* co_ln_g; const float* co_ln_b;
    const float* ff1_w; const float* ff1_b;
    const float* ff2_w; const float* ff2_b; const float* ff_ln_g; const float* ff_ln_b;
} hirest_caption_layer;
typedef struct hirest_caption_decoder {
    int32_t layers, heads, hidden, inter, vocab_padded, max_pos;
    const float* word_emb; const float* pos_emb; const float* emb_ln_g; const float* emb_ln_b;
    const hirest_caption_layer* layer;
    const float* tr_w; const float* tr_b; const float* tr_ln_g; const float* tr_ln_b;
    const float* lm_w; const float* lm_b;
    const hirest_bf16* lm_w2;
} hirest_caption_decoder;
size_t hirest_caption_step_workspace_bytes(const hirest_caption_decoder* d, int32_t R);
int hirest_caption_decode_step(const hirest_caption_decoder* d, int32_t R, int32_t position, const int32_t* last_ids,
                               const int32_t* parent_rows, const float* const* kv_in, float* const* kv_out,
                               const float* const* enc_kv, int32_t F, const float* row_add, float* logp,
                               void* workspace, size_t workspace_bytes, void* stream);

int hirest_attention_f32_decode(const float* q, int64_t ldq, const float* k_hist, const float* v_hist, int64_t ld_hist,
                                const int32_t* parent, int32_t t_hist, const float* k_new, const float* v_new, int64_t ld_new,
                                float* k_out, float* v_out, float* out, int32_t R, int32_t H, float scale, float add_const,
                                float causal_penalty, void* stream);
int hirest_caption_select(int32_t mode);
int hirest_caption_decode_logits(const hirest_caption_decoder* d, int32_t R, int32_t position, const int32_t* last_ids,
                                 const int32_t* parent_rows, const float* const* kv_in, float* const* kv_out,
                                 const float* const* enc_kv, int32_t F, float* logits, void* workspace, size_t workspace_bytes,
                                 void* stream);
size_t hirest_caption_beam_tail_workspace_bytes(int32_t B, int32_t beam, int32_t vocab);
int hirest_caption_beam_tail(const float* logits, int64_t ldx, const float* row_add, int32_t B, int32_t beam, int32_t vocab,
                             int32_t step, int32_t max_steps, int32_t eos_id, float* scores, int32_t* tokens, int32_t* backptr,
                             int32_t* n_steps, int32_t* done, int32_t* next_ids, int32_t* next_parents, float* next_add,
                             int32_t* done_host, void* workspace, size_t workspace_bytes, void* stream);

int hirest_caption_beam_step(const hirest_caption_decoder* d, int32_t B, int32_t beam, int32_t position, int32_t* ids, int32_t* parent_rows,
                             const float* const* kv_in, float* const* kv_out, const float* const* enc_kv, int32_t F, float* row_add,
                             float* logits, int32_t max_steps, int32_t eos_id, float* scores, int32_t* tokens, int32_t* backptr,
                             int32_t* n_steps, int32_t* done, int32_t* done_host, void* workspace, size_t workspace_bytes,
                             void* tail_workspace, size_t tail_workspace_bytes, void* stream);

int hirest_beam_advance(const float* val, const int32_t* idx, int32_t B, int32_t beam, int32_t vocab, int32_t step, int32_t max_steps,
                        int32_t eos_id, float* scores, int32_t* tokens, int32_t* backptr, int32_t* n_steps, int32_t* done,
                        int32_t* next_ids, int32_t* next_parents, float* next_add, void* stream);
int hirest_beam_backtrack(const float* scores, const int32_t* tokens, const int32_t* backptr, const int32_t* n_steps, int32_t B,
                          int32_t beam, int32_t max_steps, int32_t* out, void* stream);

int hirest_gemm_f32_strided(const float* A, int64_t sam, int64_t sak, const float* B, int64_t sbn, int64_t sbk, float* C, int64_t ldc,
                            int32_t M, int32_t N, int32_t K, float alpha, void* stream);
int hirest_transpose_pad_f32(const float* in, int64_t ld_in, int32_t R, int32_t C, float* out, int32_t Rp, void* stream);
int hirest_weighted_colsum_f32(const float* x, int64_t ldx, const float* row_weight, const int32_t* row_select,
                               int32_t select_value, int32_t R, int32_t C, float* out, void* stream);
#define HIREST_COLSUM_GROUP_MAX 40
typedef struct hirest_colsum_item {
    const float*   x;
    const float*   row_weight;
    const int32_t* row_select;
    float*         out;
    int64_t        ldx;
    int32_t        R, C, select_value, reserved;
} hirest_colsum_item;
int hirest_weighted_colsum_grouped_f32(const hirest_colsum_item* items, int32_t count, void* stream);
int hirest_act_f32(const float* pre, float* y, int64_t n, int32_t act, void* stream);
int hirest_scale_by_device_scalar_f32(float* x, const float* scalar, int64_t n, void* stream);
int hirest_act_bwd_f32(const float* pre, const float* dy, float* dx, int64_t n, int32_t act, void* stream);
int hirest_dropout_add_f32(const float* x, const float* resid, float* y, int64_t n, float p, uint32_t seed, void* stream);
int hirest_layernorm_bwd_f32(const float* x, const float* dy, const float* gamma, float eps, float* dx, float* dyxhat,
                             int32_t R, int32_t D, void* stream);
int hirest_attention_train_fwd_f32(const float* qkv, float* P, float* ctx, int32_t B, int32_t T, int32_t H, int32_t dh,
                                   float scale, float add_const, float drop_p, uint32_t seed, void* stream);
int hirest_attention_train_bwd_f32(const float* qkv, const float* P, const float* dctx, float* dS, float* dqkv, int32_t B,
                                   int32_t T, int32_t H, int32_t dh, float scale, float drop_p, uint32_t seed, void* stream);
int hirest_attention_train_select(int32_t which);
int hirest_attention_train_fwd_qkv_f32(const float* q, int64_t ldq, const float* k, const float* v, int64_t ldkv,
                                       const float* mask_add, float* P, float* ctx, int64_t ldctx, int32_t B, int32_t Tq, int32_t Tk,
                                       int32_t H, int32_t dh, float scale, float add_const, float drop_p, uint32_t seed, void* stream);
int hirest_attention_train_bwd_qkv_f32(const float* q, int64_t ldq, const float* k, const float* v, int64_t ldkv, const float* P,
                                       const float* dctx, int64_t ldctx, float* dS, float* dq, int64_t lddq, float* dk, float* dv,
                                       int64_t lddkv, int32_t B, int32_t Tq, int32_t Tk, int32_t H, int32_t dh, float scale,
                                       float drop_p, uint32_t seed, void* stream);
int hirest_embedding_fwd_f32(const int32_t* ids, const float* table, const float* pos, float* out, int64_t rows, int32_t T,
                             int32_t D, void* stream);
int hirest_embedding_pos_fwd_f32(const int32_t* ids, const int32_t* pos_ids, const float* table, const float* pos, float* out,
                                 int64_t rows, int32_t D, void* stream);
int hirest_embedding_bwd_f32(const int32_t* ids, const float* dx, float* dtable_accum, int64_t rows, int32_t D, void* stream);
int hirest_ce_rows_f32(const float* logits, int64_t ld, const int32_t* target, int32_t R, int32_t V, float weight, int32_t n_valid,
                       float* loss_accum, float* dlogits, void* stream);
int hirest_bce_masked_f32(const float* logits, const int32_t* target, const int32_t* mask, int32_t B, int32_t T, float weight,
                          float* loss_accum, float* dlogits, void* stream);
int hirest_joint_base_bwd_f32(const float* dbase, const float* v, const float* tn, float* dv, float* dtn, int32_t B, int32_t T,
                              int32_t E, void* stream);
int hirest_l2norm_bwd_f32(const float* t, const float* dtn, float* dt, int32_t B, int32_t E, void* stream);
int hirest_ce_masked_f32(const float* logits, const int32_t* mask, const int32_t* target, int32_t B, int32_t T, float weight,
                         float* loss_accum, float* dlogits, void* stream);
int hirest_heads_bwd_f32(const float* dlogits, int64_t rows, int32_t D, int32_t nheads, const float* w0, const float* w1,
                         const float* w2, float* dfeats, void* stream);

int hirest_masked_argmax(const float* logits, const int32_t* mask, float fill, int32_t B, int32_t T, int32_t* out,
                         void* stream);
int hirest_moment_valid_f32(const float* logits, const int32_t* vis_mask, const int32_t* moment_mask, const int32_t* start_target,
                            const int32_t* end_target, int32_t B, int32_t T, float fill, int32_t* pred , float* loss,
                            void* stream);
size_t hirest_lm_head_ce_workspace_bytes(int32_t R, int32_t V);
int hirest_lm_head_ce_f32(const float* h, int64_t ldh, const float* W, int64_t ldw, const float* bias, const int32_t* target, int32_t R,
                          int32_t V, int32_t K, int32_t n_valid, float* nll, float* loss, void* workspace, size_t workspace_bytes,
                          void* stream);
int hirest_segmentation_step(const float* logits, int32_t* moment_mask, int32_t* boundary_mask, int32_t B, int32_t T,
                             double threshold, int32_t* steps, int32_t* nsteps, int32_t max_steps, float* probs_out,
                             void* stream);

int64_t hirest_preprocess_plan_bytes(int32_t in_h, int32_t in_w, int32_t size);
int hirest_preprocess_plan(int32_t in_h, int32_t in_w, int32_t size, void* host_plan, int64_t plan_bytes);
int64_t hirest_preprocess_workspace_bytes(int32_t in_h, int32_t in_w, int32_t size, int32_t B);
int hirest_preprocess_u8(const uint8_t* frames, int32_t B, int32_t in_h, int32_t in_w, int32_t size,
                         const void* plan_dev, void* out, int32_t out_kind, const float* mean3, const float* std3,
                         void* workspace, int64_t workspace_bytes, void* stream);

enum hirest_jpeg_reason {
    HIREST_JPEG_OK = 0, HIREST_JPEG_NOT_JPEG = 1, HIREST_JPEG_PROGRESSIVE = 2, HIREST_JPEG_ARITHMETIC = 3,
    HIREST_JPEG_LOSSLESS = 4,
    HIREST_JPEG_PRECISION = 5,
    HIREST_JPEG_COLOR = 6,
    HIREST_JPEG_SAMPLING = 7, HIREST_JPEG_MULTI_SCAN = 8,
    HIREST_JPEG_TRUNCATED = 9,
    HIREST_JPEG_BAD_TABLES = 10, HIREST_JPEG_SIZE = 11
};
#define HIREST_JPEG_ST_BAD_CODE 1
#define HIREST_JPEG_ST_COEF_OVERRUN 2
#define HIREST_JPEG_ST_OUT_OF_DATA 4
#define HIREST_JPEG_ST_BAD_RESTART 8
#define HIREST_JPEG_ST_UNSUPPORTED 16

typedef struct {
    int32_t width, height, ncomp, hs, vs;
    int32_t restart_interval, mcux, mcuy;
    int32_t supported, reason;
    int64_t scan_begin, scan_end;
    int32_t table_set, reserved;
    int64_t data_offset, out_offset;
    int64_t ws_offset, plane_offset;
} hirest_jpeg_image;

typedef struct {
    uint16_t qt[3][64];
    uint8_t huff_bits[6][16];
    uint8_t huff_vals[6][256];
} hirest_jpeg_tables;

int hirest_jpeg_parse(const uint8_t* data, int64_t size, hirest_jpeg_image* img, hirest_jpeg_tables* tables);
int64_t hirest_jpeg_workspace_bytes(hirest_jpeg_image* imgs, int32_t n);
int hirest_jpeg_decode(const hirest_jpeg_image* imgs_host, const hirest_jpeg_image* imgs_dev, int32_t n,
                       const hirest_jpeg_tables* tables_dev, const uint8_t* data, uint8_t* out, int32_t* status,
                       void* workspace, int64_t workspace_bytes, void* stream);
int hirest_jpeg_decode_host(const hirest_jpeg_image* img, const hirest_jpeg_tables* tables, const uint8_t* data,
                            uint8_t* out, int32_t* status);
int64_t hirest_jpeg_chunked_workspace_bytes(int32_t n);
int hirest_jpeg_decode_chunked(const hirest_jpeg_image* imgs_host, const hirest_jpeg_image* imgs_dev, int32_t n,
                               const hirest_jpeg_tables* tables_dev, const uint8_t* data, uint8_t* out, int32_t* status,
                               void* workspace, int64_t workspace_bytes, int64_t chunk_bytes, void* chunk_workspace,
                               int64_t chunk_workspace_bytes, void* stream);
int hirest_jpeg_decode_host_chunked(const hirest_jpeg_image* img, const hirest_jpeg_tables* tables, const uint8_t* data,
                                    int64_t chunk_bytes, uint8_t* out, int32_t* status, int32_t* rounds_out);

int hirest_interval_iou_f64(const double* a, const double* b, int64_t n, double* iou, void* stream);
int hirest_step_bound_pr(const double* refs, const int32_t* ref_off, const double* preds, const int32_t* pred_off,
                         int32_t V, double tiou, double* recall, double* precision, double* best_iou, void* stream);
int hirest_preprocess_moment_bounds(const double* preds, const int32_t* pred_off, const double* gt_minmax, int32_t V,
                                    double* out, int32_t* out_count, int32_t max_out, void* stream);

int hirest_frame_to_timestamp(const int64_t* frame, const double* duration, const int32_t* n_frames, int32_t n_frames_all,
                              int64_t per_video, int64_t n, int64_t* timestamp, void* stream);
int hirest_timestamp_to_frame(const double* t, const double* duration, const int32_t* n_frames, int32_t n_frames_all,
                              int64_t per_video, int64_t n, int64_t* frame, void* stream);

int hirest_cascade_moment_bounds(const int32_t* pred_frames, const double* duration, const int32_t* n_frames, int32_t n_frames_all,
                                 int32_t B, int32_t T, int64_t* bounds_ts, int32_t* bound_frames, int32_t* moment_mask,
                                 int32_t* boundary_mask, void* stream);
int hirest_cascade_boundaries(const int32_t* steps, const int32_t* nsteps, const int32_t* bound_frames, const double* duration,
                              const int32_t* n_frames, int32_t n_frames_all, int32_t B, int32_t iters, int32_t* n_bounds,
                              int32_t* bounds, int64_t* step_ts, int32_t* step_frames, int32_t* step_sample, int32_t* offsets,
                              void* stream);
int hirest_cascade_trim_gather(const float* vis, const float* asr, const int32_t* step_frames, const int32_t* step_sample, int32_t S,
                               int32_t B, int32_t T, int32_t D, int32_t Da, int32_t F, float* out_vis, float* out_asr, void* stream);

enum hirest_prof_kind { HIREST_PROF_GEMM = 0, HIREST_PROF_ATTENTION = 1, HIREST_PROF_LAYERNORM = 2 };
typedef struct hirest_prof_record {
    int32_t kind;
    int32_t tag;
    int64_t d0, d1, d2;
    float ms;
} hirest_prof_record;
int hirest_profile_enable(int32_t on);
int hirest_profile_collect(hirest_prof_record* out, int32_t max_records);

typedef struct hirest_joint_layer_x3 {
    const hirest_bf16* qkv_w2; const float* qkv_b;
    const hirest_bf16* ao_w2;  const float* ao_b;
    const float* ln1_g; const float* ln1_b;
    const hirest_bf16* fc1_w2; const float* fc1_b;
    const hirest_bf16* fc2_w2; const float* fc2_b;
    const float* ln2_g; const float* ln2_b;
} hirest_joint_layer_x3;
typedef struct hirest_joint_encoder_x3 {
    uint64_t struct_size;
    int32_t layers, heads, width, mlp_dim, in_dim, max_pos;
    float ln_eps, attn_shift;
    const hirest_bf16* emb_w2; const float* emb_b;
    const float* pos;
    const float* emb_ln_g; const float* emb_ln_b;
    const hirest_joint_layer_x3* layer;
} hirest_joint_encoder_x3;
size_t hirest_joint_encoder_x3_workspace_bytes(const hirest_joint_encoder_x3* e, int32_t B, int32_t T);
int hirest_joint_encoder_x3_forward(const hirest_joint_encoder_x3* e, const float* f, int32_t B, int32_t T, float* out,
                                    void* workspace, size_t workspace_bytes, void* stream);
int hirest_layernorm_f32_split2(const float* x, int64_t ldx, const float* add, int32_t period, const float* gamma, const float* beta, float eps,
                                float* out32, int64_t ldo32, hirest_bf16* out2, int64_t ldo2, int32_t rows, int32_t D, void* stream);


typedef struct hirest_train_block {
    uint64_t struct_size;
    int32_t B, T, heads, width, mlp, precision;
    float ln_eps, drop;
    uint32_t seed_attn, seed_ao, seed_out, reserved;
    const float *wqkv, *bqkv;
    const float *wo, *bo, *ln1_g, *ln1_b;
    const float *w1, *b1, *w2, *b2, *ln2_g, *ln2_b;
    const float* x;
    float *qkv, *P, *cx, *a_pre, *aa, *hpre, *hh, *x_pre, *out;
    const hirest_bf16* x2; hirest_bf16* out2;
    const hirest_bf16 *wqkv2, *wo2, *w12, *w22;
    const hirest_bf16 *wqkvT2, *woT2, *w1T2, *w2T2;
    void* ws; size_t ws_bytes;
} hirest_train_block;
typedef struct hirest_train_block_grads {
    uint64_t struct_size;
    const float* dout;
    float* dx;
    float *g_wqkv, *g_wo, *g_w1, *g_w2;
    float *g_bqkv, *g_bo, *g_b1, *g_b2, *g_ln1_g, *g_ln1_b, *g_ln2_g, *g_ln2_b;
    hirest_colsum_item* items; int32_t* n_items; int32_t max_items, reserved;
    void* side_stream; void* side_ws; size_t side_ws_bytes;
    void* scratch; size_t scratch_bytes;
} hirest_train_block_grads;
typedef struct hirest_train_fusion_bwd {
    uint64_t struct_size;
    int32_t B, T, E, W, vis_dim, text_dim, asr_dim, boundary, max_pos, reserved;
    float drop; uint32_t seed_emb;
    const float *w_emb, *emb_ln_g, *t2_w, *asr1_w, *asr0_g, *norm_g;
    const float *x0, *f, *v, *tn, *tin, *a0, *asr2, *v0, *vis2, *t, *text;
    const int32_t *mm32, *bm32, *n_valid;
    const float* dx;
    float *g_emb_ln_g, *g_emb_ln_b, *g_pos, *g_w_emb, *g_b_emb, *g_mask, *g_bound, *g_t2_w, *g_t2_b, *g_t0_w, *g_t0_b,
          *g_asr1_w, *g_asr1_b, *g_asr0_g, *g_asr0_b, *g_norm_g, *g_norm_b, *g_vis_w, *g_vis_b, *g_text_w, *g_text_b;
    hirest_colsum_item* items; int32_t* n_items; int32_t max_items, reserved2;
    void* ws; size_t ws_bytes;
    void* side_stream; void* side_ws; size_t side_ws_bytes;
    void* scratch; size_t scratch_bytes;
} hirest_train_fusion_bwd;
size_t hirest_train_fusion_backward_scratch_bytes(const hirest_train_fusion_bwd* f);
int hirest_train_fusion_backward(const hirest_train_fusion_bwd* f, void* stream);
size_t hirest_train_block_forward_scratch_bytes(const hirest_train_block* b);
int hirest_train_block_forward(const hirest_train_block* b, void* scratch, size_t scratch_bytes, void* stream);
size_t hirest_train_block_backward_scratch_bytes(const hirest_train_block* b);
int hirest_train_block_backward(const hirest_train_block* b, const hirest_train_block_grads* g, void* stream);

#define HIREST_OPTIM_GROUP_MAX 64
#define HIREST_OPTIM_CHUNK 8192
typedef struct hirest_optim_item {
    float*       p;
    const float* g;
    float*       m;
    float*       v;
    int64_t      n;
} hirest_optim_item;
int64_t hirest_optim_partials_count(const hirest_optim_item* items, int32_t count);
int hirest_grad_sqnorm_grouped_f32(const hirest_optim_item* items, int32_t count, float* partials, void* stream);
int hirest_clip_coef_f32(const float* partials, int64_t count, float max_norm, float* norm_coef, void* stream);
int hirest_adamw_grouped_f32(const hirest_optim_item* items, int32_t count, const float* coef, float decay, float one_minus_beta1,
                             float beta2, float one_minus_beta2, float step_size, float bc2_sqrt, float eps, void* stream);
int hirest_grad_sqnorm_scaled_grouped_f32(const hirest_optim_item* items, int32_t count, const float* grad_scale, float* partials,
                                          void* stream);
int hirest_clip_coef_dev_f32(const float* partials, int64_t count, const float* max_norm, float* norm_coef, void* stream);
int hirest_optim_step_advance_f32(float* const* steps, int32_t count, const float* found_inf, void* stream);
int hirest_adamw_capturable_grouped_f32(const hirest_optim_item* items, float* const* steps, int32_t count, const float* coef,
                                        const float* lr_ptr, double lr, const float* grad_scale, const float* found_inf,
                                        double beta1, double beta2, float eps, double weight_decay, void* stream);

#define HIREST_BATCH_GATHER_MAX 8
typedef struct hirest_batch_gather {
    const void* src;
    void*       dst;
    const int32_t* row_of_example;
    int32_t words, reserved;
} hirest_batch_gather;
typedef struct hirest_batch_args {
    uint64_t struct_size;
    const int32_t* index;
    int32_t B, T, D, Da, n_examples, n_model_frames, n_gather, reserved;
    const float*   frames;
    const int64_t* frame_off;
    const float*   asr_rows;
    const int64_t* sub_off;
    const int32_t* sub_span;
    const int32_t* ex_video;
    const int32_t* ex_len;
    const int32_t* ex_range;
    const int32_t* bound_off;
    const int32_t* bound_val;
    float*   vis;
    float*   asr;
    int64_t *vis_mask, *moment_mask, *prev_boundary_mask;
    hirest_batch_gather gather[HIREST_BATCH_GATHER_MAX];
} hirest_batch_args;
int hirest_batch_assemble(const hirest_batch_args* a, void* stream);

#ifdef __cplusplus
}
#endif
#endif
```

Measured before the change: 2094.

## Add store-in-flight attention variant with team-based head/frame block mapping

Adds a new default attention variant (8) built from a shared kernel body. It drops the per-step vmcnt(0) wait for compute waves so output stores and next-Q loads stay in flight across steps. It zero-masks Q padding in registers, specializes the head loop by which query tiles a wave owns, and adds a 'team' mapping in which each block walks a subset of heads across frames (auto team 4 for large batches). The aim is to overlap global stores and loads with compute and to improve L2 locality and load balance. The cost is more template complexity and possible register pressure.

```diff
diff --git a/hirest_amd/_lib.py b/hirest_amd/_lib.py
--- a/hirest_amd/_lib.py
+++ b/hirest_amd/_lib.py
@@ -205,6 +205,7 @@
     "hirest_attention_select_kernel": (C.c_int, [C.c_int32]),
     "hirest_attention_set_skew": (C.c_int, [C.c_int32]),
     "hirest_attention_set_mapping": (C.c_int, [C.c_int32]),
+    "hirest_attention_set_team": (C.c_int, [C.c_int32]),
     "hirest_attention_set_pace": (C.c_int, [C.c_int32]),
     "hirest_attention_x3_select_waves": (C.c_int, [C.c_int32]),
     "hirest_attention_x3_debug_trace": (C.c_int, [C.c_void_p]),
@@ -439,6 +440,8 @@
         fn.restype, fn.argtypes = res, args
     if os.environ.get("HIREST_ATTENTION_KERNEL"):
         check(lib.hirest_attention_select_kernel(int(os.environ["HIREST_ATTENTION_KERNEL"])), "HIREST_ATTENTION_KERNEL")
+    if os.environ.get("HIREST_ATTENTION_TEAM"):
+        check(lib.hirest_attention_set_team(int(os.environ["HIREST_ATTENTION_TEAM"])), "HIREST_ATTENTION_TEAM")
     _lib = lib
     return lib
 
diff --git a/hirest_amd/csrc/attention.hip b/hirest_amd/csrc/attention.hip
--- a/hirest_amd/csrc/attention.hip
+++ b/hirest_amd/csrc/attention.hip
@@ -1,6 +1,8 @@
 #include "common.h"
 #include <atomic>
+#include <type_traits>
 #include "profile.h"
+#include "gemm_shared.h"
 
 namespace {
 
@@ -308,10 +310,11 @@
     return r;
 }
 typedef float f32x2_t __attribute__((ext_vector_type(2)));
-template <int DH, int DP, int NT, bool FAST, bool DBG, int NW = 9, bool LEAN = false, bool PROD = false>
-__global__ __launch_bounds__((NW + (PROD ? 1 : 0)) * 64) void attention_kernel_v3(const bf16_t* __restrict__ qkv, bf16_t* __restrict__ out,
+template <int DH, int DP, int NT, bool FAST, bool DBG, int NW = 9, bool LEAN = false, bool PROD = false, bool INFLIGHT = false>
+__device__ __forceinline__ void attention_v3_body(const bf16_t* __restrict__ qkv, bf16_t* __restrict__ out,
                                                           int N, int H, float scale_log2e, int causal, int dbg_bits, int nq, int skew,
-                                                          int B, int map, int pace, int stagger) {
+                                                          int B, int map, int pace, int stagger, int team) {
+    static_assert(!INFLIGHT || (PROD && !DBG), "the compute waves of the store-in-flight form issue no LDS-DMA and carry no timing switches");
     const int dbg = DBG ? dbg_bits : 0;
     using C = AttnCfg2<DH, DP, NT>;
     extern __shared__ __attribute__((aligned(16))) char smem[];
@@ -323,13 +326,15 @@
     int b0, bstep, h0, hstep, nsteps;
     if (map == 0) { b0 = blockIdx.x; bstep = 0; h0 = 0; hstep = 1; nsteps = H; }
     else {
-        const int xcd = blockIdx.x & 7, slot = blockIdx.x >> 3, FL = (gridDim.x >> 3) / H;
-        h0 = slot % H; hstep = 0; b0 = xcd * FL + slot / H; bstep = 8 * FL;
-        nsteps = b0 < B ? (B - b0 + bstep - 1) / bstep : 0;
+        const int xcd = blockIdx.x & 7, slot = blockIdx.x >> 3, TL = (gridDim.x >> 3) / team;
+        h0 = slot % team; hstep = team; b0 = xcd * TL + slot / team; bstep = 8 * TL;
+        nsteps = b0 < B ? (B - b0 + bstep - 1) / bstep * (H / team) : 0;
     }
     if (nsteps == 0) return;
-    if (stagger > 0 && blockIdx.x < 256) sleep_n(((blockIdx.x >> 3) & 15) * stagger);
-    auto sbase = [&](int st) { return qkv + (int64_t)(b0 + st * bstep) * N * ld + (h0 + st * hstep) * DH; };
+    if (stagger > 0 && blockIdx.x < 256) sleep_n((map == 2 ? (((blockIdx.x >> 3) / team * team) >> 1) & 15 : (blockIdx.x >> 3) & 15) * stagger);
+    struct Pos { int f, hd; };
+    auto next_pos = [&](Pos p) { p.hd += hstep; if (p.hd >= H) { p.hd = h0; p.f += bstep; } return p; };
+    auto sbase = [&](Pos p) { return qkv + (int64_t)p.f * N * ld + p.hd * DH; };
     const int g = lane >> 4, c16 = lane & 15;
     const int gk = g ^ ((-(c16 >> 2)) & 3);
     const int nqt = (nq + 15) >> 4;
@@ -342,9 +347,9 @@
     static_assert(ROWS_PER_PIECE_OK<NW, C::CPR>::value, "a lane's rows must keep (row >> 2) & 1 from piece to piece");
     static_assert((NW * 64) % C::CPR == 0, "piece stride must be whole rows");
     constexpr int ROWS_PER_PIECE = NW * 64 / C::CPR;
-    auto dma_k = [&](int h, char* dst) -> int {
+    auto dma_k = [&](Pos ps, char* dst) -> int {
         int n = 0;
-        const bf16_t* src = sbase(h) + D;
+        const bf16_t* src = sbase(ps) + D;
         for (int i = wave, row = row0; i < C::NK_INSTR; i += NW, row += ROWS_PER_PIECE) {
             int kc = (col0 & ~3) | ((col0 & 3) ^ ((-(row >> 2)) & 3));
             const bool kpad = kc * 8 >= DH;
@@ -359,8 +364,8 @@
     };
     constexpr bool SUM_IN_MFMA = LEAN && DP > DH;
     const bool vpad = SUM_IN_MFMA && vlog * 8 >= DH;
-    auto dma_v = [&](int h) {
-        const bf16_t* src = sbase(h) + 2 * D + vc * 8;
+    auto dma_v = [&](Pos ps) {
+        const bf16_t* src = sbase(ps) + 2 * D + vc * 8;
         for (int i = wave, row = row0; i < C::NV_INSTR; i += NW, row += ROWS_PER_PIECE) {
             const int r = row < N ? row : N - 1;
             const void* from = src + (int64_t)r * ld;
@@ -368,10 +373,19 @@
             glds16(from, Vs + i * 1024);
         }
     };
-    auto load_q = [&](int h, int qtile, bf16x8 (&dst)[DP / 32]) {
+    auto load_q = [&](Pos ps, int qtile, bf16x8 (&dst)[DP / 32]) {
         const int q = qtile * 16 + c16;
-        const bf16_t* base = sbase(h);
+        const bf16_t* base = sbase(ps);
         if (LEAN && DP > DH) {
+            const bf16_t* row = base + (int64_t)(q < N ? q : N - 1) * ld;
+#pragma unroll
+            for (int kk = 0; kk < DP / 32; ++kk) {
+                const int d = (kk * 4 + g) * 8;
+                dst[kk] = *reinterpret_cast<const bf16x8*>(row + (d < DH ? d : DH - 8));
+            }
+            return;
+        }
+        if (INFLIGHT) {
             const bf16_t* row = base + (int64_t)(q < N ? q : N - 1) * ld;
 #pragma unroll
             for (int kk = 0; kk < DP / 32; ++kk) {
@@ -405,8 +419,8 @@
             pvpad[j] = SUM_IN_MFMA && vl * 8 >= DH;
             pvoff[j] = (vl * 8 < DH ? vl : DH / 8 - 1) * 8;
         }
-        auto issue_k = [&](int st, char* dst, int pace_units) {
-            const bf16_t* src = sbase(st) + D;
+        auto issue_k = [&](Pos ps, char* dst, int pace_units) {
+            const bf16_t* src = sbase(ps) + D;
             for (int it0 = 0; it0 < C::NK_INSTR / PER; ++it0) {
                 const int it = map ? (it0 + h0) % (C::NK_INSTR / PER) : it0;
 #pragma unroll
@@ -419,8 +433,8 @@
                 }
             }
         };
-        auto issue_v = [&](int st) {
-            const bf16_t* src = sbase(st) + 2 * D;
+        auto issue_v = [&](Pos ps) {
+            const bf16_t* src = sbase(ps) + 2 * D;
             for (int it0 = 0; it0 < C::NV_INSTR / PER; ++it0) {
                 const int it = map ? (it0 + h0) % (C::NV_INSTR / PER) : it0;
 #pragma unroll
@@ -432,195 +446,242 @@
                 }
             }
         };
-        issue_k(0, smem, 0);
+        Pos cur = {b0, h0};
+        issue_k(cur, smem, 0);
         for (int h = 0; h < nsteps; ++h) {
             asm volatile("s_waitcnt vmcnt(0)" ::: "memory");
             __builtin_amdgcn_s_barrier();
-            issue_v(h);
+            issue_v(cur);
             asm volatile("s_waitcnt vmcnt(0)" ::: "memory");
             __builtin_amdgcn_s_barrier();
-            if (h + 1 < nsteps) issue_k(h + 1, smem + ((h + 1) & 1) * (C::NPAD * C::RS), pace);
+            cur = next_pos(cur);
+            if (h + 1 < nsteps) issue_k(cur, smem + ((h + 1) & 1) * (C::NPAD * C::RS), pace);
         }
         asm volatile("s_waitcnt vmcnt(0)" ::: "memory");
         return;
     }
 
-    bf16x8 qa[DP / 32], qb[DP / 32];
-    load_q(0, wave, qa);
-    load_q(0, wave + NW, qb);
-    if (!(dbg & 8) && !PROD) dma_k(0, smem);
-    for (int h = 0; h < nsteps; ++h) {
-        const char* Ks = smem + (h & 1) * (C::NPAD * C::RS);
-        auto stamp = [&](int slot) {
-            if (DBG && (dbg & 256) && blockIdx.x == 0 && h < ATTN_TRACE_STEPS) {
-                const long long t = __builtin_readcyclecounter();
-                if (lane == 0) g_attn_trace[(h * ATTN_TRACE_WAVES + wave) * ATTN_TRACE_SLOTS + slot] = t;
-            }
-        };
-        stamp(10);
-        asm volatile("s_waitcnt vmcnt(0)" ::: "memory");
+    bf16x8 qa[DP / 32] = {}, qb[DP / 32] = {};
+    Pos cur = {b0, h0};
+    const bool has_a = wave < nqt, has_b = wave + NW < nqt;
+    if (!INFLIGHT || has_a) load_q(cur, wave, qa);
+    if (!INFLIGHT || has_b) load_q(cur, wave + NW, qb);
+    if (!(dbg & 8) && !PROD) dma_k(cur, smem);
+    if (INFLIGHT) {
 #pragma unroll
         for (int kk = 0; kk < DP / 32; ++kk) { asm volatile("" : "+v"(qa[kk])); asm volatile("" : "+v"(qb[kk])); }
-        if (!(dbg & 128)) __builtin_amdgcn_s_barrier();
-        stamp(0);
-        if (!(dbg & 8) && !PROD) dma_v(h);
-        const int nk_next = (h + 1 < nsteps && !(dbg & 8) && !PROD) ? dma_k(h + 1, smem + ((h + 1) & 1) * (C::NPAD * C::RS)) : 0;
-        bool v_ready = false;
-        auto tile = [&](int qt, bf16x8 (&qf)[DP / 32], int ord) {
-            stamp(1 + 4 * ord);
-            const int q = qt * 16 + c16;
-            const bool qvalid = q < N;
-            f32x4 st[NT];
-#pragma unroll
-            for (int t = 0; t < NT; t += 2) {
-                f32x4 a0 = {0.f, 0.f, 0.f, 0.f}, a1 = {0.f, 0.f, 0.f, 0.f};
-                if (!(dbg & 1))
-#pragma unroll
-                for (int kk = 0; kk < DP / 32; ++kk) {
-                    const bf16x8 k0 = *reinterpret_cast<const bf16x8*>(Ks + (t * 16 + c16) * C::RS + (kk * 4 + gk) * 16);
-                    a0 = __builtin_amdgcn_mfma_f32_16x16x32_bf16(k0, qf[kk], a0, 0, 0, 0);
-                    if (t + 1 < NT) {
-                        const bf16x8 k1 = *reinterpret_cast<const bf16x8*>(Ks + ((t + 1) * 16 + c16) * C::RS + (kk * 4 + gk) * 16);
-                        a1 = __builtin_amdgcn_mfma_f32_16x16x32_bf16(k1, qf[kk], a1, 0, 0, 0);
+    }
+    auto head_loop = [&](auto mode_c) {
+        constexpr int MODE = decltype(mode_c)::value;
+        for (int h = 0; h < nsteps; ++h, cur = next_pos(cur)) {
+            const char* Ks = smem + (h & 1) * (C::NPAD * C::RS);
+            const Pos nxt = next_pos(cur);
+            const Pos qnext = h + 1 < nsteps ? nxt : cur;
+            const __amdgpu_buffer_rsrc_t orsrc = hx_rsrc(out + (int64_t)cur.f * N * D + cur.hd * DH, ((unsigned)(N - 1) * (unsigned)D + (unsigned)DH) * 2u);
+            auto stamp = [&](int slot) {
+                if (DBG && (dbg & 256) && blockIdx.x == 0 && h < ATTN_TRACE_STEPS) {
+                    const long long t = __builtin_readcyclecounter();
+                    if (lane == 0) g_attn_trace[(h * ATTN_TRACE_WAVES + wave) * ATTN_TRACE_SLOTS + slot] = t;
+                }
+            };
+            stamp(10);
+            if (!INFLIGHT) {
+                asm volatile("s_waitcnt vmcnt(0)" ::: "memory");
+#pragma unroll
+                for (int kk = 0; kk < DP / 32; ++kk) { asm volatile("" : "+v"(qa[kk])); asm volatile("" : "+v"(qb[kk])); }
+            }
+            if (!(dbg & 128)) __builtin_amdgcn_s_barrier();
+            stamp(0);
+            if (!(dbg & 8) && !PROD) dma_v(cur);
+            const int nk_next = (h + 1 < nsteps && !(dbg & 8) && !PROD) ? dma_k(nxt, smem + ((h + 1) & 1) * (C::NPAD * C::RS)) : 0;
+            bool v_ready = false;
+            auto tile = [&](int qt, bf16x8 (&qf)[DP / 32], int ord) {
+                stamp(1 + 4 * ord);
+                const int q = qt * 16 + c16;
+                const bool qvalid = q < N;
+                if (INFLIGHT && !(LEAN && DP > DH)) {
+#pragma unroll
+                    for (int kk = 0; kk < DP / 32; ++kk) {
+                        const bool keep = qvalid && (kk * 4 + g) * 8 < DH;
+                        u32x4 w = __builtin_bit_cast(u32x4, qf[kk]);
+#pragma unroll
+                        for (int e = 0; e < 4; ++e) w[e] = keep ? w[e] : 0u;
+                        qf[kk] = __builtin_bit_cast(bf16x8, w);
                     }
                 }
-                st[t] = a0;
-                if (t + 1 < NT) st[t + 1] = a1;
-                if ((t & 2) || !FAST) __builtin_amdgcn_sched_barrier(0);
-            }
-            if (h + 1 < nsteps && !(dbg & 32)) load_q(h + 1, qt, qf);
-            stamp(2 + 4 * ord);
-            const int klimit = causal ? (q < N - 1 ? q : N - 1) : N - 1;
-            float mx = -3.0e38f;
-            float sum = 0.f;
-            bf16x8 pf[C::KS];
-            if (LEAN) {
-                float mxb = -3.0e38f;
+                f32x4 st[NT];
+#pragma unroll
+                for (int t = 0; t < NT; t += 2) {
+                    f32x4 a0 = {0.f, 0.f, 0.f, 0.f}, a1 = {0.f, 0.f, 0.f, 0.f};
+                    if (!(dbg & 1))
+#pragma unroll
+                    for (int kk = 0; kk < DP / 32; ++kk) {
+                        const bf16x8 k0 = *reinterpret_cast<const bf16x8*>(Ks + (t * 16 + c16) * C::RS + (kk * 4 + gk) * 16);
+                        a0 = __builtin_amdgcn_mfma_f32_16x16x32_bf16(k0, qf[kk], a0, 0, 0, 0);
+                        if (t + 1 < NT) {
+                            const bf16x8 k1 = *reinterpret_cast<const bf16x8*>(Ks + ((t + 1) * 16 + c16) * C::RS + (kk * 4 + gk) * 16);
+                            a1 = __builtin_amdgcn_mfma_f32_16x16x32_bf16(k1, qf[kk], a1, 0, 0, 0);
+                        }
+                    }
+                    st[t] = a0;
+                    if (t + 1 < NT) st[t + 1] = a1;
+                    if ((t & 2) || !FAST) __builtin_amdgcn_sched_barrier(0);
+                }
+                if (INFLIGHT) load_q(qnext, qt, qf);
+                else if (h + 1 < nsteps && !(dbg & 32)) load_q(nxt, qt, qf);
+                stamp(2 + 4 * ord);
+                const int klimit = causal ? (q < N - 1 ? q : N - 1) : N - 1;
+                float mx = -3.0e38f;
+                float sum = 0.f;
+                bf16x8 pf[C::KS];
+                if (LEAN) {
+                    float mxb = -3.0e38f;
+#pragma unroll
+                    for (int t = 0; t < NT; ++t) {
+                        if (!FAST || t == NT - 1) {
+#pragma unroll
+                            for (int i = 0; i < 4; ++i) st[t][i] = (t * 16 + 4 * g + i) <= klimit ? st[t][i] : -3.0e38f;
+                        }
+                        if (t & 1) { mxb = max3_raw(mxb, st[t][0], st[t][1]); mxb = max3_raw(mxb, st[t][2], st[t][3]); }
+                        else { mx = max3_raw(mx, st[t][0], st[t][1]); mx = max3_raw(mx, st[t][2], st[t][3]); }
+                    }
+                    float pa = max3_raw(mx, mxb, mxb), pb = pa;
+                    lane_swap16(pa, pb); pa = max3_raw(pa, pb, pb); pb = pa; lane_swap32(pa, pb); mx = max3_raw(pa, pb, pb);
+                    const float nmc = -mx * scale_log2e;
+                    const f32x2_t sc2 = {scale_log2e, scale_log2e}, nm2 = {nmc, nmc};
+                    f32x2_t sum2 = {0.f, 0.f};
+#pragma unroll
+                    for (int s2 = 0; s2 < C::KS; ++s2) {
+#pragma unroll
+                        for (int u = 0; u < 2; ++u) {
+                            if (2 * s2 + u < NT) {
+#pragma unroll
+                                for (int ip = 0; ip < 2; ++ip) {
+                                    const f32x2_t sv = {st[2 * s2 + u][2 * ip], st[2 * s2 + u][2 * ip + 1]};
+                                    const f32x2_t e = __builtin_elementwise_fma(sv, sc2, nm2);
+                                    const f32x2_t p2 = (dbg & 2) ? e : f32x2_t{__builtin_amdgcn_exp2f(e[0]), __builtin_amdgcn_exp2f(e[1])};
+                                    if (!SUM_IN_MFMA) sum2 += p2;
+                                    pf[s2][4 * u + 2 * ip] = (bf16_t)p2[0];
+                                    pf[s2][4 * u + 2 * ip + 1] = (bf16_t)p2[1];
+                                }
+                            } else {
+#pragma unroll
+                                for (int i = 0; i < 4; ++i) pf[s2][4 + i] = (bf16_t)0.f;
+                            }
+                        }
+                    }
+                    if (!SUM_IN_MFMA) {
+                        sum = sum2[0] + sum2[1];
+                        float sa = sum, sb = sum; lane_swap16(sa, sb); sum = sa + sb; sa = sum; sb = sum; lane_swap32(sa, sb); sum = sa + sb;
+                    }
+                } else {
 #pragma unroll
                 for (int t = 0; t < NT; ++t) {
                     if (!FAST || t == NT - 1) {
 #pragma unroll
                         for (int i = 0; i < 4; ++i) st[t][i] = (t * 16 + 4 * g + i) <= klimit ? st[t][i] : -3.0e38f;
                     }
-                    if (t & 1) { mxb = max3_raw(mxb, st[t][0], st[t][1]); mxb = max3_raw(mxb, st[t][2], st[t][3]); }
-                    else { mx = max3_raw(mx, st[t][0], st[t][1]); mx = max3_raw(mx, st[t][2], st[t][3]); }
-                }
-                float pa = max3_raw(mx, mxb, mxb), pb = pa;
-                lane_swap16(pa, pb); pa = max3_raw(pa, pb, pb); pb = pa; lane_swap32(pa, pb); mx = max3_raw(pa, pb, pb);
+                    mx = fmaxf(fmaxf(mx, fmaxf(st[t][0], st[t][1])), fmaxf(st[t][2], st[t][3]));
+                }
+                { float pa = mx, pb = mx; lane_swap16(pa, pb); mx = fmaxf(pa, pb); pa = mx; pb = mx; lane_swap32(pa, pb); mx = fmaxf(pa, pb); }
                 const float nmc = -mx * scale_log2e;
-                const f32x2_t sc2 = {scale_log2e, scale_log2e}, nm2 = {nmc, nmc};
-                f32x2_t sum2 = {0.f, 0.f};
 #pragma unroll
                 for (int s2 = 0; s2 < C::KS; ++s2) {
 #pragma unroll
-                    for (int u = 0; u < 2; ++u) {
-                        if (2 * s2 + u < NT) {
-#pragma unroll
-                            for (int ip = 0; ip < 2; ++ip) {
-                                const f32x2_t sv = {st[2 * s2 + u][2 * ip], st[2 * s2 + u][2 * ip + 1]};
-                                const f32x2_t e = __builtin_elementwise_fma(sv, sc2, nm2);
-                                const f32x2_t p2 = (dbg & 2) ? e : f32x2_t{__builtin_amdgcn_exp2f(e[0]), __builtin_amdgcn_exp2f(e[1])};
-                                if (!SUM_IN_MFMA) sum2 += p2;
-                                pf[s2][4 * u + 2 * ip] = (bf16_t)p2[0];
-                                pf[s2][4 * u + 2 * ip + 1] = (bf16_t)p2[1];
-                            }
+                    for (int i = 0; i < 4; ++i) {
+                        const float e0 = fmaf(st[2 * s2][i], scale_log2e, nmc);
+                        const float p0 = (dbg & 2) ? e0 : __builtin_amdgcn_exp2f(e0);
+                        sum += p0;
+                        pf[s2][i] = (bf16_t)p0;
+                        if (2 * s2 + 1 < NT) {
+                            const float e1 = fmaf(st[2 * s2 + 1][i], scale_log2e, nmc);
+                            const float p1 = (dbg & 2) ? e1 : __builtin_amdgcn_exp2f(e1);
+                            sum += p1;
+                            pf[s2][4 + i] = (bf16_t)p1;
                         } else {
-#pragma unroll
-                            for (int i = 0; i < 4; ++i) pf[s2][4 + i] = (bf16_t)0.f;
+                            pf[s2][4 + i] = (bf16_t)0.f;
                         }
                     }
                 }
-                if (!SUM_IN_MFMA) {
-                    sum = sum2[0] + sum2[1];
-                    float sa = sum, sb = sum; lane_swap16(sa, sb); sum = sa + sb; sa = sum; sb = sum; lane_swap32(sa, sb); sum = sa + sb;
-                }
-            } else {
-#pragma unroll
-            for (int t = 0; t < NT; ++t) {
-                if (!FAST || t == NT - 1) {
-#pragma unroll
-                    for (int i = 0; i < 4; ++i) st[t][i] = (t * 16 + 4 * g + i) <= klimit ? st[t][i] : -3.0e38f;
-                }
-                mx = fmaxf(fmaxf(mx, fmaxf(st[t][0], st[t][1])), fmaxf(st[t][2], st[t][3]));
-            }
-            { float pa = mx, pb = mx; lane_swap16(pa, pb); mx = fmaxf(pa, pb); pa = mx; pb = mx; lane_swap32(pa, pb); mx = fmaxf(pa, pb); }
-            const float nmc = -mx * scale_log2e;
-#pragma unroll
-            for (int s2 = 0; s2 < C::KS; ++s2) {
-#pragma unroll
-                for (int i = 0; i < 4; ++i) {
-                    const float e0 = fmaf(st[2 * s2][i], scale_log2e, nmc);
-                    const float p0 = (dbg & 2) ? e0 : __builtin_amdgcn_exp2f(e0);
-                    sum += p0;
-                    pf[s2][i] = (bf16_t)p0;
-                    if (2 * s2 + 1 < NT) {
-                        const float e1 = fmaf(st[2 * s2 + 1][i], scale_log2e, nmc);
-                        const float p1 = (dbg & 2) ? e1 : __builtin_amdgcn_exp2f(e1);
-                        sum += p1;
-                        pf[s2][4 + i] = (bf16_t)p1;
-                    } else {
-                        pf[s2][4 + i] = (bf16_t)0.f;
+                { float pa = sum, pb = sum; lane_swap16(pa, pb); sum = pa + pb; pa = sum; pb = sum; lane_swap32(pa, pb); sum = pa + pb; }
+                }
+                stamp(3 + 4 * ord);
+                if (!v_ready) {
+                    if (!PROD) wait_vm_le(nk_next);
+                    if (!(dbg & 64)) __builtin_amdgcn_s_barrier();
+                    v_ready = true;
+                }
+                stamp(4 + 4 * ord);
+                const char* vlane = Vs + (4 * g + (c16 >> 2)) * C::RS + (c16 & 3) * 8;
+                const char* vl_e = vlane + ((VSWAP && (g & 1)) ? 32 : 0);
+                const char* vl_o = vlane - ((VSWAP && (g & 1)) ? 32 : 0);
+                f32x4 oacc[DP / 16];
+#pragma unroll
+                for (int dt = 0; dt < DP / 16; ++dt) oacc[dt] = f32x4{0.f, 0.f, 0.f, 0.f};
+                if (!(dbg & 4))
+#pragma unroll
+                for (int s2 = 0; s2 < C::KS; ++s2) {
+#pragma unroll
+                    for (int dt = 0; dt < DP / 16; ++dt) {
+                        const char* vrow = ((dt & 1) ? vl_o : vl_e) + dt * 32 + s2 * 32 * C::RS;
+                        const bf16x4 lo = __builtin_amdgcn_ds_read_tr16_b64_v4bf16((__attribute__((address_space(3))) bf16x4*)(vrow));
+                        const bf16x4 hi = __builtin_amdgcn_ds_read_tr16_b64_v4bf16((__attribute__((address_space(3))) bf16x4*)(vrow + 16 * C::RS));
+                        const bf16x8 vf = {lo[0], lo[1], lo[2], lo[3], hi[0], hi[1], hi[2], hi[3]};
+                        oacc[dt] = __builtin_amdgcn_mfma_f32_16x16x32_bf16(vf, pf[s2], oacc[dt], 0, 0, 0);
                     }
-                }
-            }
-            { float pa = sum, pb = sum; lane_swap16(pa, pb); sum = pa + pb; pa = sum; pb = sum; lane_swap32(pa, pb); sum = pa + pb; }
-            }
-            stamp(3 + 4 * ord);
+                    if ((s2 & 1) || !FAST) __builtin_amdgcn_sched_barrier(0);
+                }
+                if (SUM_IN_MFMA) {
+                    float sa = oacc[DP / 16 - 1][0], sb = sa;
+                    lane_swap32(sa, sb);
+                    sum = sb;
+                }
+                const float inv = 1.0f / sum;
+                static_assert((DP / 16) % 2 == 0 && DH % 8 == 0, "paired d tiles");
+#pragma unroll
+                for (int dp = 0; dp < DP / 32; ++dp) {
+                    union { bf16x4 v; unsigned u[2]; } e, o;
+#pragma unroll
+                    for (int i = 0; i < 4; ++i) { e.v[i] = (bf16_t)(oacc[2 * dp][i] * inv); o.v[i] = (bf16_t)(oacc[2 * dp + 1][i] * inv); }
+                    const auto s0 = __builtin_amdgcn_permlane16_swap(e.u[0], o.u[0], false, false);
+                    const auto s1 = __builtin_amdgcn_permlane16_swap(e.u[1], o.u[1], false, false);
+                    union { bf16x8 v; unsigned u[4]; } w;
+                    w.u[0] = s0[0]; w.u[1] = s1[0]; w.u[2] = s0[1]; w.u[3] = s1[1];
+                    const int d = (2 * dp + (g & 1)) * 16 + (g >> 1) * 8;
+                    if (INFLIGHT) {
+                        const u32x4 wu = {w.u[0], w.u[1], w.u[2], w.u[3]};
+                        __builtin_amdgcn_raw_buffer_store_b128(wu, orsrc, (qvalid && d < DH) ? (unsigned)(q * D + d) * 2u : HX_OOB, 0, 0);
+                    } else if (qvalid && d < DH && !(dbg & 16)) *reinterpret_cast<bf16x8*>(out + ((int64_t)cur.f * N + q) * D + cur.hd * DH + d) = w.v;
+                }
+            };
+            if (skew > 0 && wave >= 4 && wave < 8) sleep_n(skew);
+            if (MODE == 0 ? has_a : MODE != 3) tile(wave, qa, 0);
+            if (MODE == 0 ? has_b : MODE == 2) tile(wave + NW, qb, 1);
+            stamp(9);
             if (!v_ready) {
                 if (!PROD) wait_vm_le(nk_next);
-                if (!(dbg & 64)) __builtin_amdgcn_s_barrier();
-                v_ready = true;
-            }
-            stamp(4 + 4 * ord);
-            const char* vlane = Vs + (4 * g + (c16 >> 2)) * C::RS + (c16 & 3) * 8;
-            const char* vl_e = vlane + ((VSWAP && (g & 1)) ? 32 : 0);
-            const char* vl_o = vlane - ((VSWAP && (g & 1)) ? 32 : 0);
-            f32x4 oacc[DP / 16];
-#pragma unroll
-            for (int dt = 0; dt < DP / 16; ++dt) oacc[dt] = f32x4{0.f, 0.f, 0.f, 0.f};
-            if (!(dbg & 4))
-#pragma unroll
-            for (int s2 = 0; s2 < C::KS; ++s2) {
-#pragma unroll
-                for (int dt = 0; dt < DP / 16; ++dt) {
-                    const char* vrow = ((dt & 1) ? vl_o : vl_e) + dt * 32 + s2 * 32 * C::RS;
-                    const bf16x4 lo = __builtin_amdgcn_ds_read_tr16_b64_v4bf16((__attribute__((address_space(3))) bf16x4*)(vrow));
-                    const bf16x4 hi = __builtin_amdgcn_ds_read_tr16_b64_v4bf16((__attribute__((address_space(3))) bf16x4*)(vrow + 16 * C::RS));
-                    const bf16x8 vf = {lo[0], lo[1], lo[2], lo[3], hi[0], hi[1], hi[2], hi[3]};
-                    oacc[dt] = __builtin_amdgcn_mfma_f32_16x16x32_bf16(vf, pf[s2], oacc[dt], 0, 0, 0);
-                }
-                if ((s2 & 1) || !FAST) __builtin_amdgcn_sched_barrier(0);
-            }
-            if (SUM_IN_MFMA) {
-                float sa = oacc[DP / 16 - 1][0], sb = sa;
-                lane_swap32(sa, sb);
-                sum = sb;
-            }
-            const float inv = 1.0f / sum;
-            static_assert((DP / 16) % 2 == 0 && DH % 8 == 0, "paired d tiles");
-#pragma unroll
-            for (int dp = 0; dp < DP / 32; ++dp) {
-                union { bf16x4 v; unsigned u[2]; } e, o;
-#pragma unroll
-                for (int i = 0; i < 4; ++i) { e.v[i] = (bf16_t)(oacc[2 * dp][i] * inv); o.v[i] = (bf16_t)(oacc[2 * dp + 1][i] * inv); }
-                const auto s0 = __builtin_amdgcn_permlane16_swap(e.u[0], o.u[0], false, false);
-                const auto s1 = __builtin_amdgcn_permlane16_swap(e.u[1], o.u[1], false, false);
-                union { bf16x8 v; unsigned u[4]; } w;
-                w.u[0] = s0[0]; w.u[1] = s1[0]; w.u[2] = s0[1]; w.u[3] = s1[1];
-                const int d = (2 * dp + (g & 1)) * 16 + (g >> 1) * 8;
-                if (qvalid && d < DH && !(dbg & 16)) *reinterpret_cast<bf16x8*>(out + ((int64_t)(b0 + h * bstep) * N + q) * D + (h0 + h * hstep) * DH + d) = w.v;
-            }
-        };
-        if (skew > 0 && wave >= 4 && wave < 8) sleep_n(skew);
-        if (wave < nqt) tile(wave, qa, 0);
-        if (wave + NW < nqt) tile(wave + NW, qb, 1);
-        stamp(9);
-        if (!v_ready) {
-            if (!PROD) wait_vm_le(nk_next);
-            __builtin_amdgcn_s_barrier();
-        }
-    }
+                __builtin_amdgcn_s_barrier();
+            }
+        }
+    };
+    if constexpr (!INFLIGHT) head_loop(std::integral_constant<int, 0>{});
+    else if (has_b) head_loop(std::integral_constant<int, 2>{});
+    else if (has_a) head_loop(std::integral_constant<int, 1>{});
+    else head_loop(std::integral_constant<int, 3>{});
     asm volatile("s_waitcnt vmcnt(0)" ::: "memory");
+}
+
+template <int DH, int DP, int NT, bool FAST, bool DBG, int NW = 9, bool LEAN = false, bool PROD = false>
+__global__ __launch_bounds__((NW + (PROD ? 1 : 0)) * 64) void attention_kernel_v3(const bf16_t* __restrict__ qkv, bf16_t* __restrict__ out,
+                                                          int N, int H, float scale_log2e, int causal, int dbg_bits, int nq, int skew,
+                                                          int B, int map, int pace, int stagger, int team) {
+    attention_v3_body<DH, DP, NT, FAST, DBG, NW, LEAN, PROD, false>(qkv, out, N, H, scale_log2e, causal, dbg_bits, nq, skew, B, map, pace, stagger, team);
+}
+template <int DH, int DP, int NT, bool FAST>
+__global__ __launch_bounds__(640) void attention_kernel_v3s(const bf16_t* __restrict__ qkv, bf16_t* __restrict__ out,
+                                                          int N, int H, float scale_log2e, int causal, int dbg_bits, int nq, int skew,
+                                                          int B, int map, int pace, int stagger, int team) {
+    attention_v3_body<DH, DP, NT, FAST, false, 9, false, true, true>(qkv, out, N, H, scale_log2e, causal, dbg_bits, nq, skew, B, map, pace, stagger, team);
 }
 
 std::atomic<int> g_attn_dbg{0};
@@ -628,25 +689,40 @@
 std::atomic<int> g_attn_stagger{16};
 std::atomic<int> g_attn_pace{0};
 std::atomic<int> g_attn_map{2};
-std::atomic<int> g_attn_variant{7};
-
-template <int DH, int DP, int NT, bool FAST, bool DBG, int NW = 9, bool LEAN = false, bool PROD = false>
+std::atomic<int> g_attn_variant{8};
+std::atomic<int> g_attn_team{0};
+constexpr int ATTN_TEAM_AUTO = 4;
+
+template <int DH, int DP, int NT, bool FAST, bool DBG, int NW = 9, bool LEAN = false, bool PROD = false, bool INFLIGHT = false>
 int launch3_impl(const bf16_t* qkv, bf16_t* out, int B, int N, int H, float scale, int causal, int nq, hipStream_t s) {
     using C = AttnCfg2<DH, DP, NT>;
     constexpr int LDS = (2 * C::NPAD + C::KP) * C::RS;
     static_assert(LDS <= 163840, "K x2 + V must fit the CU's LDS");
     static HirestDevCfg cfg;
-    auto kern = attention_kernel_v3<DH, DP, NT, FAST, DBG, NW, LEAN, PROD>;
+    auto kern = [] {
+        if constexpr (INFLIGHT) return attention_kernel_v3s<DH, DP, NT, FAST>;
+        else return attention_kernel_v3<DH, DP, NT, FAST, DBG, NW, LEAN, PROD>;
+    }();
     if (int e = hirest_configure(kern, LDS, cfg)) return e;
+    auto team_fits = [&](int t) { return t >= 2 && t <= 32 && H % t == 0 && 32 % t == 0; };
     const bool by_head = (g_attn_map == 1 || (g_attn_map == 2 && B < 256)) && H <= 32 && 32 % H == 0 && B >= 8 * (32 / H) * 4;
-    const int grid = by_head ? 256 : B;
+    int map = by_head ? 1 : 0, team = by_head ? H : 1;
+    const int asked = g_attn_team;
+    if (team_fits(asked)) { map = 2; team = asked; }
+    else if (INFLIGHT && g_attn_map == 2 && B >= 256) {
+        int t = ATTN_TEAM_AUTO;
+        while (t >= 2 && !team_fits(t)) t >>= 1;
+        if (t >= 2) { map = 2; team = t; }
+    }
+    const int grid = map ? 256 : B;
     hipLaunchKernelGGL(kern, dim3(grid), dim3((NW + (PROD ? 1 : 0)) * 64), LDS, s, qkv, out, N, H, scale * 1.44269504088896340736f, causal, g_attn_dbg, nq,
-                       g_attn_skew, B, by_head ? 1 : 0, g_attn_pace, g_attn_stagger);
+                       g_attn_skew, B, map, g_attn_pace, g_attn_stagger, team);
     return hirest_launch_status();
 }
 
 template <int DH, int DP, int NT, bool FAST>
 int launch3(const bf16_t* qkv, bf16_t* out, int B, int N, int H, float scale, int causal, int nq, hipStream_t s) {
+    if (g_attn_variant == 8) return launch3_impl<DH, DP, NT, FAST, false, 9, false, true, true>(qkv, out, B, N, H, scale, causal, nq, s);
     if (g_attn_dbg && FAST && g_attn_variant == 6) return launch3_impl<DH, DP, NT, FAST, true, 9, true, true>(qkv, out, B, N, H, scale, causal, nq, s);
     if (g_attn_variant == 6) return launch3_impl<DH, DP, NT, FAST, false, 9, true, true>(qkv, out, B, N, H, scale, causal, nq, s);
     if (g_attn_dbg && FAST && g_attn_variant == 7) return launch3_impl<DH, DP, NT, FAST, true, 9, false, true>(qkv, out, B, N, H, scale, causal, nq, s);
@@ -702,8 +778,14 @@
     return 0;
 }
 
+extern "C" int hirest_attention_set_team(int32_t team) {
+    if (team != 0 && team != 2 && team != 4 && team != 8 && team != 16) return HIREST_E_BADARG;
+    g_attn_team = team;
+    return 0;
+}
+
 extern "C" int hirest_attention_select_kernel(int32_t which) {
-    if (which < 1 || which > 7) return HIREST_E_BADARG;
+    if (which < 1 || which > 8) return HIREST_E_BADARG;
     g_attn_variant = which;
     return 0;
 }
diff --git a/hirest_amd/ops.py b/hirest_amd/ops.py
--- a/hirest_amd/ops.py
+++ b/hirest_amd/ops.py
@@ -74,7 +74,7 @@
     _lib.check(_lib.load().hirest_gemm_select_kernel(int(which)), "hirest_gemm_select_kernel")
 
 
-ATTENTION_DEFAULT_KERNEL = 7
+ATTENTION_DEFAULT_KERNEL = 8
 
 
 def attention_select_kernel(which: int):
@@ -83,6 +83,10 @@
 
 def attention_set_mapping(by_head: Optional[bool] = None):
     _lib.check(_lib.load().hirest_attention_set_mapping(2 if by_head is None else int(bool(by_head))), "hirest_attention_set_mapping")
+
+
+def attention_set_team(team: int = 0):
+    _lib.check(_lib.load().hirest_attention_set_team(int(team)), "hirest_attention_set_team")
 
 
 @on_tensor_device
diff --git a/include/hirest_hip.h b/include/hirest_hip.h
--- a/include/hirest_hip.h
+++ b/include/hirest_hip.h
@@ -70,6 +70,7 @@
                                float scale, int32_t causal, int32_t q_rows, void* stream);
 int hirest_attention_select_kernel(int32_t which);
 int hirest_attention_set_mapping(int32_t by_head);
+int hirest_attention_set_team(int32_t team);
 int hirest_attention_set_pace(int32_t units);
 int hirest_attention_set_stagger(int32_t units);
 int hirest_attention_set_skew(int32_t units);
```

New measurement: 2100, median of 6. About the same (+0.3%).
